# DJATOM/x265-aMod

Measured on AMD Instinct MI355X. Metric: encoded frames/sec at 1080p & 2160p --preset medium; bit-exact vs CPU ref, higher is better.
Workload: dtype u8

## Files before the change

### x265-amod_amd/csrc/encoder_api.hip

```cpp
#include "encoder_impl.h"

extern "C" void x265amd_param_default(x265amd_param* p)
{
    if (!p) return;
    memset(p, 0, sizeof(*p));
    p->fpsNum = 25; p->fpsDenom = 1;
    p->bframes = 0; p->keyframeMax = 250; p->maxNumReferences = 3; p->qp = 30; p->ipFactor = 1.4f; p->pbFactor = 1.3f;
    p->rateControlMode = X265AMD_RC_CQP; p->rfConstant = 28; p->aqStrength = 1.0; p->qCompress = 0.6; p->aqMode = 0; p->cuTree = 0; p->qgSize = 32; p->qpMin = 0; p->qpMax = 69; p->vuiVideoFormat = 5; p->vuiColorPrimaries = 2; p->vuiTransfer = 2; p->vuiMatrix = 2; p->bEmitCLL = 1;
    p->rdLevel = 3; p->limitReferences = 3; p->bEnableEarlySkip = 1; p->recursionSkipMode = 1; p->bIntraInBFrames = 1; p->psyRd = 2.0; p->edgeVarThreshold = 0.05f;
    p->searchMethod = X265AMD_ME_HEX; p->subpelRefine = 2; p->searchRange = 57; p->maxNumMergeCand = 3;
    p->bEnableSignHiding = 1; p->bEnableStrongIntraSmoothing = 1; p->bEnableTemporalMvp = 1; p->tuQTMaxInterDepth = 1; p->tuQTMaxIntraDepth = 1;
    p->bEnableLoopFilter = 1; p->bEnableSAO = 1; p->bEnableWavefront = 1; p->aspectRatioIdc = 0;
}

void x265amd_encoder::fillStreamParams(x265amd_stream_params& s) const
{
    memset(&s, 0, sizeof(s));
    static const struct { uint32_t maxLumaSamples, maxLumaSamplesPerSecond; int idc; } levels[] = {
        { 36864, 552960, 30 }, { 122880, 3686400, 60 }, { 245760, 7372800, 63 }, { 552960, 16588800, 90 }, { 983040, 33177600, 93 },
        { 2228224, 66846720, 120 }, { 2228224, 133693440, 123 }, { 8912896, 267386880, 150 }, { 8912896, 534773760, 153 },
        { 8912896, 1069547520, 156 }, { 35651584, 1069547520, 180 }, { 35651584, 2139095040u, 183 }, { 35651584, 4278190080u, 186 } };
    s.profile_idc = X265AMD_DEPTH <= 8 ? 1 : 2;
    s.profile_compatibility_flags = X265AMD_DEPTH <= 8 ? (1u << 1) | (1u << 2) : (1u << 2);
    s.progressive_source = 1; s.frame_only_constraint = 1;
    s.bit_depth_constraint = X265AMD_DEPTH; s.chroma_format_constraint = 1; s.lower_bit_rate_constraint = 1;
    s.intra_constraint = p.keyframeMax <= 1;
    if (s.intra_constraint) { s.profile_idc = 4; s.profile_compatibility_flags = 1u << 4; }
    const uint32_t lumaSamples = (uint32_t)(W * H);
    const uint32_t samplesPerSec = (uint32_t)(lumaSamples * ((double)p.fpsNum / p.fpsDenom));
    s.level_idc = 255;
    for (const auto& l : levels)
    {
        if (lumaSamples > l.maxLumaSamples || samplesPerSec > l.maxLumaSamplesPerSecond) continue;
        if (W > sqrt(l.maxLumaSamples * 8.0f) || H > sqrt(l.maxLumaSamples * 8.0f)) continue;
        uint32_t maxDpbSize = 6;
        if (lumaSamples <= (l.maxLumaSamples >> 2)) maxDpbSize = 16;
        else if (lumaSamples <= (l.maxLumaSamples >> 1)) maxDpbSize = 12;
        else if (lumaSamples <= ((3 * l.maxLumaSamples) >> 2)) maxDpbSize = 8;
        if ((uint32_t)maxDecPicBuffering > maxDpbSize) continue;
        s.level_idc = l.idc;
        break;
    }
    s.max_temporal_sub_layers = 1;
    s.max_dec_pic_buffering[0] = maxDecPicBuffering; s.num_reorder_pics[0] = numReorderPics; s.max_latency_increase[0] = p.bframes;
    s.chroma_format_idc = 1; s.pic_width = W; s.pic_height = H; s.bit_depth = X265AMD_DEPTH; s.log2_max_poc_lsb = 8;
    s.conformance_window = W != srcW || H != srcH; s.conf_win_offsets[1] = W - srcW; s.conf_win_offsets[3] = H - srcH;
    s.log2_min_cu_size = 3; s.log2_diff_max_min_cu_size = 3; s.tu_log2_min = 2; s.tu_log2_max = 5;
    s.tu_max_depth_inter = p.tuQTMaxInterDepth; s.tu_max_depth_intra = p.tuQTMaxIntraDepth;
    s.amp = p.bEnableAMP != 0; s.sao = p.bEnableSAO != 0; s.temporal_mvp = p.bEnableTemporalMvp != 0; s.strong_intra_smoothing = p.bEnableStrongIntraSmoothing != 0;
    s.aspect_ratio_idc = p.aspectRatioIdc; s.sar_width = p.vuiSarWidth; s.sar_height = p.vuiSarHeight;
    s.overscan_info_present = p.vuiOverscanInfoPresent != 0; s.overscan_appropriate = p.vuiOverscanAppropriate != 0;
    s.video_signal_type_present = p.vuiVideoSignalTypePresent != 0; s.video_format = p.vuiVideoFormat; s.video_full_range = p.vuiFullRange != 0;
    s.colour_description_present = p.vuiColorDescriptionPresent != 0; s.colour_primaries = p.vuiColorPrimaries; s.transfer_characteristics = p.vuiTransfer; s.matrix_coefficients = p.vuiMatrix;
    s.chroma_loc_info_present = p.vuiChromaLocPresent != 0; s.chroma_sample_loc_top = p.vuiChromaLocTop; s.chroma_sample_loc_bottom = p.vuiChromaLocBottom;
    s.default_display_window = p.vuiDisplayWindow != 0;
    s.def_disp_win_offsets[0] = p.vuiDispWinLeft; s.def_disp_win_offsets[1] = p.vuiDispWinRight; s.def_disp_win_offsets[2] = p.vuiDispWinTop; s.def_disp_win_offsets[3] = p.vuiDispWinBottom;
    s.emit_timing_info = 1; s.num_units_in_tick = p.fpsDenom; s.time_scale = p.fpsNum;
    s.weighted_pred = p.bEnableWeightedPred != 0; s.weighted_bipred = p.bEnableWeightedBiPred != 0;
    s.sign_hide = p.bEnableSignHiding != 0; s.num_ref_idx_default[0] = s.num_ref_idx_default[1] = 1; s.init_qp_minus26 = 0;
    s.use_dqp = useDqp; s.max_cu_dqp_depth = maxCuDqpDepth;
    s.wpp = p.bEnableWavefront != 0; s.loop_filter_across_slices = 1;
    s.deblocking_filter_control_present = !p.bEnableLoopFilter || p.deblockingFilterBetaOffset || p.deblockingFilterTCOffset; s.pic_disable_deblocking = !p.bEnableLoopFilter;
    s.beta_offset_div2 = p.deblockingFilterBetaOffset; s.tc_offset_div2 = p.deblockingFilterTCOffset;
}

extern "C" x265amd_encoder* x265amd_encoder_open(const x265amd_param* p)
{
    if (!p) { xa_fail(X265AMD_EINVAL, "encoder_open: null param"); return nullptr; }
    x265amd_param norm = *p;
    if (norm.keyframeMax < 0) { norm.keyframeMax = INT_MAX; norm.scenecutThreshold = 0; norm.bHistBasedSceneCut = 0; }
    if (norm.keyframeMax <= 1 && norm.keyframeMax >= 0)
    {
        norm.keyframeMax = 1; norm.keyframeMin = 1; norm.bFrameAdaptive = 0; norm.bframes = 0; norm.bOpenGOP = 0; norm.bRepeatHeaders = 1; norm.lookaheadDepth = 0;
        norm.scenecutThreshold = 0; norm.bHistBasedSceneCut = 0; norm.cuTree = 0; norm.bEnableWeightedPred = 0; norm.bEnableWeightedBiPred = 0; norm.maxNumReferences = 1;
    }
    if (norm.bEmitHDR10SEI || norm.hasMasteringDisplay || norm.maxCLL || norm.maxFALL) { norm.bEmitHDR10SEI = 1; norm.bRepeatHeaders = 1; }
    if (norm.limitTU && norm.tuQTMaxInterDepth < 2) norm.limitTU = 0;
    if (norm.rateControlMode != X265AMD_RC_CRF) { norm.aqMode = 0; norm.cuTree = 0; }
    if (norm.lookaheadDepth == 0) norm.cuTree = 0;
    if (!norm.aqMode && norm.cuTree) { norm.aqMode = 1; norm.aqStrength = 0.0; }
    if (norm.aqStrength == 0 && !norm.cuTree) norm.aqMode = 0;
    if ((((norm.sourceHeight + 7) & ~7) + 63) / 64 == 1 || (((norm.sourceWidth + 7) & ~7) + 63) / 64 < 3) norm.bEnableWavefront = 0;
    p = &norm;
    if (p->sourceWidth < 16 || p->sourceHeight < 16 || (p->sourceWidth & 1) || (p->sourceHeight & 1) || p->sourceWidth > 8192 || p->sourceHeight > 4320)
    { xa_fail(X265AMD_EINVAL, "encoder_open: picture size must be even (4:2:0) and within 16..8192 x 16..4320"); return nullptr; }
    if (p->sourceWidth <= 64 && p->sourceHeight <= 64)
    { xa_fail(X265AMD_EINVAL, "encoder_open: sourceWidth / sourceHeight: a picture of a single CTU is not built"); return nullptr; }
    {
        static thread_local char why[160];
        const char* bad = nullptr;
#define XA_REQUIRE(cond, text) do { if (!bad && !(cond)) bad = text; } while (0)
        XA_REQUIRE(p->fpsNum && p->fpsDenom, "fpsNum / fpsDenom must be non-zero");
        XA_REQUIRE(p->bframes >= 0 && p->bframes <= 16, "bframes outside 0..16");
        XA_REQUIRE(p->keyframeMax >= 1, "keyframeMax below 1");
        XA_REQUIRE(p->maxNumReferences >= 1 && p->maxNumReferences <= 8, "maxNumReferences outside 1..8");
        XA_REQUIRE(p->rateControlMode == 0 || p->rateControlMode == X265AMD_RC_CQP || p->rateControlMode == X265AMD_RC_CRF, "rc.rateControlMode: constant QP (1) and constant rate factor (2) are built, ABR (0 with a bitrate) is not");
        XA_REQUIRE(p->rateControlMode == X265AMD_RC_CRF || (p->qp >= 0 && p->qp <= 51), "qp outside 0..51");
        XA_REQUIRE(p->rateControlMode != X265AMD_RC_CRF || (p->rfConstant >= 0 && p->rfConstant <= 51), "rfConstant outside 0..51");
        XA_REQUIRE(p->aqMode >= 0 && p->aqMode <= 5, "aqMode outside 0..5");
        XA_REQUIRE(p->qpMin >= 0 && p->qpMin <= p->qpMax && p->qpMax <= 69, "qpMin / qpMax outside 0..69 (or crossed)");
        XA_REQUIRE(p->aspectRatioIdc >= 0 && (p->aspectRatioIdc <= 16 || p->aspectRatioIdc == 255), "aspectRatioIdc outside 0..16 / 255");
        XA_REQUIRE(p->deblockingFilterTCOffset >= -6 && p->deblockingFilterTCOffset <= 6 && p->deblockingFilterBetaOffset >= -6 && p->deblockingFilterBetaOffset <= 6, "deblocking offsets outside -6..6");
        XA_REQUIRE(p->limitTU == 0 || (p->limitTU >= 2 && p->limitTU <= 4), "limitTU: 0, 2, 3 and 4 are built (1, the breadth-first form, is not)");
        XA_REQUIRE(p->limitTU < 3 || p->shardCount <= 1, "limitTU 3 / 4 with pictures coded on several GPUs is not built (the transform depth records do not travel)");
        XA_REQUIRE(p->decodedPictureHashSEI >= 0 && p->decodedPictureHashSEI <= 3 && p->maxCLL >= 0 && p->maxCLL <= 65535 && p->maxFALL >= 0 && p->maxFALL <= 65535, "decodedPictureHashSEI outside 0..3 or a light level outside 16 bits");
        XA_REQUIRE(p->vuiVideoFormat >= 0 && p->vuiVideoFormat <= 5 && p->vuiColorPrimaries >= 0 && p->vuiColorPrimaries <= 255 && p->vuiTransfer >= 0 && p->vuiTransfer <= 255 &&
                   p->vuiMatrix >= 0 && p->vuiMatrix <= 255 && p->vuiChromaLocTop >= 0 && p->vuiChromaLocTop <= 5 && p->vuiChromaLocBottom >= 0 && p->vuiChromaLocBottom <= 5, "vui: a value outside its range");
        XA_REQUIRE(!p->aqMode || p->aqStrength >= 0, "aqStrength negative");
        XA_REQUIRE(!p->aqMode || p->qgSize == 32 || p->qgSize == 64, "qgSize: 64 and 32 are built");
        XA_REQUIRE(!p->cuTree || p->aqMode, "cuTree needs adaptive quantisation (Encoder::configure switches it on with cuTree; say aqMode)");
        XA_REQUIRE(!p->cuTree || p->rateControlMode == X265AMD_RC_CRF, "cuTree needs rate control (the reference switches it off under constant QP, encoder.cpp:3721-3728)");
        XA_REQUIRE(!p->cuTree || p->lookaheadDepth > 0, "cuTree needs the lookahead (lookaheadDepth > 0)");
        XA_REQUIRE(!(p->aqMode && p->rateControlMode != X265AMD_RC_CRF), "adaptive quantisation needs rate control (the reference switches it off under constant QP, encoder.cpp:3721-3728)");
        XA_REQUIRE(p->rdLevel >= 2 && p->rdLevel <= 6, "rdLevel outside 2..6 (rd 0-1 are not built)");
        XA_REQUIRE(p->maxNumMergeCand >= 1 && p->maxNumMergeCand <= 5, "maxNumMergeCand outside 1..5");
        XA_REQUIRE(p->tuQTMaxInterDepth >= 1 && p->tuQTMaxInterDepth <= 4, "tuQTMaxInterDepth outside 1..4");
        XA_REQUIRE(p->tuQTMaxIntraDepth >= 1 && p->tuQTMaxIntraDepth <= 4, "tuQTMaxIntraDepth outside 1..4");
        XA_REQUIRE(p->searchMethod == X265AMD_ME_DIA || p->searchMethod == X265AMD_ME_HEX || p->searchMethod == X265AMD_ME_STAR || p->searchMethod == X265AMD_ME_FULL, "searchMethod: only dia, hex, star and full are built (no umh / sea)");
        XA_REQUIRE(p->subpelRefine >= 0 && p->subpelRefine <= 7, "subpelRefine outside 0..7");
        XA_REQUIRE(p->rdoqLevel >= 0 && p->rdoqLevel <= 2, "rdoqLevel outside 0..2");
        XA_REQUIRE(p->psyRdoqFix8 >= 0, "psyRdoqFix8 negative");
        XA_REQUIRE(p->recursionSkipMode >= 0 && p->recursionSkipMode <= 2, "recursionSkipMode outside 0..2");
        XA_REQUIRE(p->recursionSkipMode != 2 || p->aqMode < 4, "recursionSkipMode 2 with aqMode 4 / 5 is not built (the bit plane would come from the filtered edge picture)");
        XA_REQUIRE(p->recursionSkipMode != 2 || (p->edgeVarThreshold >= 0.0f && p->edgeVarThreshold <= 1.0f), "edgeVarThreshold outside 0..1 (--rskip-edge-threshold 0..100)");
        XA_REQUIRE(p->recursionSkipMode != 2 || p->shardCount <= 1, "recursionSkipMode 2 with pictures coded on several GPUs (shardCount > 1) is not built");
        XA_REQUIRE(!p->bHistBasedSceneCut || X265AMD_DEPTH == 8, "bHistBasedSceneCut: histogram scene-cut detection is built for the 8-bit library only");
        XA_REQUIRE(!p->bHistBasedSceneCut || p->shardCount <= 1, "bHistBasedSceneCut with pictures coded on several GPUs (shardCount > 1) is not built");
        XA_REQUIRE(p->limitReferences >= 0 && p->limitReferences <= 3, "limitReferences outside 0..3");
        XA_REQUIRE(!p->bEnableAMP || p->bEnableRectInter, "bEnableAMP needs bEnableRectInter");
#undef XA_REQUIRE
        if (bad) { snprintf(why, sizeof(why), "encoder_open: %s", bad); xa_fail(X265AMD_EINVAL, why); return nullptr; }
    }
    xa_bind_device();
    std::unique_ptr<x265amd_encoder> e(new x265amd_encoder);
    e->p = *p;
    e->srcW = p->sourceWidth; e->srcH = p->sourceHeight;
    e->W = (p->sourceWidth + 7) & ~7; e->H = (p->sourceHeight + 7) & ~7; e->w4 = e->W / 4; e->h4 = e->H / 4;
    e->ctuW = (e->W + 63) / 64; e->ctuH = (e->H + 63) / 64; e->nctu = e->ctuW * e->ctuH;
    e->stride = e->W + 2 * e->marginX; e->cstride = e->W / 2 + e->marginX;
    const size_t ysz = (size_t)(e->H + 2 * e->marginY) * e->stride, csz = (size_t)(e->H / 2 + e->marginY) * e->cstride;
    e->org[0] = (size_t)e->marginY * e->stride + e->marginX;
    e->org[1] = ysz + (size_t)(e->marginY / 2) * e->cstride + e->marginX / 2;
    e->org[2] = ysz + csz + (size_t)(e->marginY / 2) * e->cstride + e->marginX / 2;
    e->picElems = ysz + 2 * csz;
    const double ipOffset = 6.0 * log2(p->ipFactor), pbOffset = 6.0 * log2(p->pbFactor);
    auto clipQp = [](int q) { return q < 0 ? 0 : q > 69 ? 69 : q; };
    e->qpConstant[1] = p->qp;
    e->qpConstant[2] = clipQp((int)(p->qp - ipOffset + 0.5));
    e->qpConstant[0] = clipQp((int)(p->qp + pbOffset + 0.5));
    if (e->qpConstant[0] > 51 || e->qpConstant[2] > 51) { xa_fail(X265AMD_EINVAL, "encoder_open: slice QP above 51"); return nullptr; }
    e->numReorderPics = (p->bBPyramid && p->bframes > 1) ? 2 : (p->bframes ? 1 : 0);
    e->maxDecPicBuffering = std::min(16, std::max(e->numReorderPics + 2, p->maxNumReferences) + 1);
    if (p->firstFrame < 0) { xa_fail(X265AMD_EINVAL, "encoder_open: firstFrame"); return nullptr; }
    e->frameCount = p->firstFrame; e->lastKeyframe = p->firstFrame - p->keyframeMax; e->lastIDR = p->firstFrame;
    if (p->scenecutThreshold < 0 || p->scenecutThreshold > 100 || p->lookaheadDepth < 0 || p->lookaheadDepth > 250 || p->keyframeMin < 0 || p->keyframeMin > p->keyframeMax)
    { xa_fail(X265AMD_EINVAL, "encoder_open: scenecutThreshold outside 0..100, lookaheadDepth outside 0..250 or keyframeMin outside 0..keyframeMax"); return nullptr; }
    if (p->shardCount < 0 || p->shardCount > 64 || (p->shardCount > 1 && (p->shardRank < 0 || p->shardRank >= p->shardCount || p->frameNumThreads <= 1)))
    { xa_fail(X265AMD_EINVAL, "encoder_open: shardRank / shardCount (frame-per-GPU needs 0 <= rank < count and frameNumThreads > 1: rows are published by pictures coded in parallel)"); return nullptr; }
    if (p->bFrameAdaptive < 0 || p->bFrameAdaptive > 2) { xa_fail(X265AMD_EINVAL, "encoder_open: bFrameAdaptive: 0 (fixed mini-GOPs), 1 (fast) or 2 (trellis)"); return nullptr; }
    e->lookahead = p->scenecutThreshold > 0 || p->bHistBasedSceneCut || (p->bFrameAdaptive && p->bframes) || p->cuTree || p->aqMode;
    x265amd_hist_scene_state_init(&e->histState);
    if ((p->bEnableWeightedPred || p->bEnableWeightedBiPred) && !e->lookahead) { xa_fail(X265AMD_EINVAL, "encoder_open: bEnableWeightedPred needs the lookahead (scenecutThreshold > 0 or bFrameAdaptive 2 with B frames)"); return nullptr; }
    {
        int kmin = p->keyframeMin;
        if (!kmin) { const double fps = (double)p->fpsNum / p->fpsDenom; kmin = std::min((int)fps, p->keyframeMax / 10); }
        e->keyframeMin = std::max(1, kmin);
        e->lowCuW = (e->W / 2 + 7) >> 3; e->lowCuH = (e->H / 2 + 7) >> 3;
        if (p->lookaheadSlices > 1 && e->H >= 720)
        {
            e->laRowsPerSlice = std::min(std::max(e->lowCuH / p->lookaheadSlices, 10), e->lowCuH);
            e->laNumSlices = e->lowCuH / e->laRowsPerSlice;
        }
        if (e->laNumSlices > 1 && p->bframes == 0 && p->lookaheadDepth > 0)
        { xa_fail(X265AMD_EINVAL, "encoder_open: bframes 0 with lookaheadSlices above 1 in a picture of 720 rows or more is not built (lookaheadSlices 0 is)"); return nullptr; }
        e->lowW = e->lowCuW * 8; e->lowH = e->lowCuH * 8;
        e->lowBlocks = (e->lowCuW > 2 && e->lowCuH > 2) ? (e->lowCuW - 2) * (e->lowCuH - 2) : e->lowCuW * e->lowCuH;
        e->lowStride = e->W / 2 + 2 * e->marginX;
        e->lowStride += (32 - (e->lowStride & 31)) & 31;
        e->lowPlaneElems = (size_t)(e->lowH + 2 * e->marginY) * e->lowStride;
        e->lowOrg = (size_t)e->marginY * e->lowStride + e->marginX;
        if (e->lookahead)
        {
            int least = 0, greatest = 0;
            if (hipDeviceGetStreamPriorityRange(&least, &greatest) != hipSuccess || least == greatest || hipStreamCreateWithPriority(&e->laStream, hipStreamNonBlocking, least) != hipSuccess)
                if (hipStreamCreateWithFlags(&e->laStream, hipStreamNonBlocking) != hipSuccess) { xa_fail(X265AMD_EHIP, "encoder_open: stream"); return nullptr; }
        }
    }
    {
        const char* ft = xa_env_str("X265AMD_FRAME_THREADS");
        e->frameThreads = ft ? atoi(ft) : 3;
        if (e->frameThreads < 1) e->frameThreads = 1;
    }
    if (p->frameNumThreads < 0 || p->frameNumThreads > 16) { xa_fail(X265AMD_EINVAL, "encoder_open: frameNumThreads"); return nullptr; }
    e->frameParallel = p->frameNumThreads > 1;
    const int queues = xa_queues_hint(0);
    if (e->frameParallel)
    {
        static const int hpelIters[8] = { 1, 1, 1, 2, 3, 1, 2, 3 };
        int range = p->searchRange;
        range += p->searchMethod < 2;
        range += 8 / 2;
        range += 2 + (hpelIters[p->subpelRefine] + 1) / 2;
        e->refLagRows = 1 + ((range + 63) / 64);
        if (!xa_env_present("X265AMD_FRAME_THREADS"))
        {
            const int rowsInFlight = p->bEnableWavefront ? std::max(1, std::min(e->ctuH, (e->ctuW + 1) / 2)) : 1;
            e->frameThreads = std::max(2, std::min(16, (queues > 0 ? queues : 16) / rowsInFlight));
        }
    }
    e->me = x265amd_me_open();
    if (!e->me) return nullptr;
    e->laPool.reset(new LaPool);
    e->laPool->one = (((size_t)e->lowCuW * e->lowCuH * 4) + 255) & ~(size_t)255;
    e->aqOn = p->aqMode != 0 && p->rateControlMode == X265AMD_RC_CRF;
    e->useDqp = e->aqOn;
    e->maxCuDqpDepth = e->aqOn ? (p->qgSize == 64 ? 0 : 1) : 0;
    memset(&e->treeParams, 0, sizeof(e->treeParams));
    e->treeParams.width8 = e->lowCuW; e->treeParams.height8 = e->lowCuH; e->treeParams.fps_num = p->fpsNum; e->treeParams.fps_denom = p->fpsDenom;
    e->treeParams.b_pyramid = p->bBPyramid != 0; e->treeParams.weighted_bipred = p->bEnableWeightedBiPred != 0; e->treeParams.lookahead_depth = p->lookaheadDepth;
    e->treeParams.strength = 5.0 * (1.0 - p->qCompress);
    if (p->rateControlMode == X265AMD_RC_CRF)
    {
        x265amd_rc_params rp;
        memset(&rp, 0, sizeof(rp));
        rp.width = e->W; rp.height = e->H; rp.fps_num = p->fpsNum; rp.fps_denom = p->fpsDenom; rp.bframes = p->bframes; rp.keyframe_max = p->keyframeMax; rp.cu_tree = p->cuTree != 0;
        rp.qp_min = p->qpMin; rp.qp_max = p->qpMax; rp.rf_constant = p->rfConstant; rp.q_compress = p->qCompress; rp.ip_factor = p->ipFactor; rp.pb_factor = p->pbFactor;
        e->rateCtl = x265amd_rc_open(&rp);
        if (!e->rateCtl) { xa_fail(X265AMD_EINVAL, "encoder_open: rate control parameters"); return nullptr; }
    }
    const size_t nstat = (size_t)e->nctu * 3 * 5 * 32;
    if (hipMalloc((void**)&e->dSaoCount, nstat * 4) != hipSuccess || hipMalloc((void**)&e->dSaoOrg, nstat * 4) != hipSuccess ||
        hipMalloc((void**)&e->dSaoParams, sizeof(x265amd_sao_ctu) * e->nctu) != hipSuccess ||
        hipMalloc((void**)&e->dDbUnits, sizeof(x265amd_deblock_unit) * e->w4 * e->h4) != hipSuccess ||
        xa_scratch_alloc((void**)&e->dSaoTmp, e->picElems * sizeof(pixel)) != hipSuccess)
    { xa_fail(X265AMD_EHIP, "encoder_open: device allocation"); return nullptr; }
    x265amd_stream_params sp;
    e->fillStreamParams(sp);
    e->headerBytes.resize(512);
    const size_t n = x265amd_write_stream_headers(&sp, e->headerBytes.data(), e->headerBytes.size());
    if (!n || n > e->headerBytes.size()) { xa_fail(X265AMD_EINVAL, "encoder_open: stream headers"); return nullptr; }
    e->headerBytes.resize(n);
    if (p->bEmitHDR10SEI || p->hasMasteringDisplay || p->maxCLL || p->maxFALL)
    {
        uint8_t sei[64], payload[24];
        if (p->bEmitCLL)
        {
            payload[0] = (uint8_t)(p->maxCLL >> 8); payload[1] = (uint8_t)p->maxCLL; payload[2] = (uint8_t)(p->maxFALL >> 8); payload[3] = (uint8_t)p->maxFALL;
            const size_t m = x265amd_write_sei(0, 144, payload, 4, sei, sizeof(sei));
            if (!m) { xa_fail(X265AMD_EINVAL, "encoder_open: content light level SEI"); return nullptr; }
            e->headerBytes.insert(e->headerBytes.end(), sei, sei + m);
        }
        if (p->hasMasteringDisplay)
        {
            for (int i = 0; i < 8; i++) { payload[2 * i] = (uint8_t)(p->masteringDisplay[i] >> 8); payload[2 * i + 1] = (uint8_t)p->masteringDisplay[i]; }
            for (int i = 0; i < 2; i++)
                for (int k = 0; k < 4; k++) payload[16 + 4 * i + k] = (uint8_t)(p->masteringDisplay[8 + i] >> (24 - 8 * k));
            const size_t m = x265amd_write_sei(0, 137, payload, 24, sei, sizeof(sei));
            if (!m) { xa_fail(X265AMD_EINVAL, "encoder_open: mastering display SEI"); return nullptr; }
            e->headerBytes.insert(e->headerBytes.end(), sei, sei + m);
        }
    }
    if (p->bEmitInfoSEI)
    {
        char text[1024];
        snprintf(text, sizeof(text), "x265amd (x265 build 209 interface) - %s - H.265/HEVC codec on AMD Instinct MI355X - options: %dx%d fps=%u/%u bitdepth=%d %s=%g aq-mode=%d aq-strength=%.2f "
                 "cutree=%d qcomp=%.2f qg-size=%d bframes=%d b-adapt=%d b-pyramid=%d open-gop=%d keyint=%d min-keyint=%d scenecut=%d rc-lookahead=%d lookahead-slices=%d ref=%d limit-refs=%d "
                 "rd=%d rdoq-level=%d psy-rd=%.2f me=%d subme=%d merange=%d max-merge=%d rect=%d amp=%d limit-modes=%d early-skip=%d rskip=%d weightp=%d weightb=%d sao=%d deblock=%d wpp=%d "
                 "tu-intra-depth=%d tu-inter-depth=%d signhide=%d strong-intra-smoothing=%d temporal-mvp=%d b-intra=%d fast-intra=%d",
                 x265amd_version(), p->sourceWidth, p->sourceHeight, p->fpsNum, p->fpsDenom, X265AMD_DEPTH, p->rateControlMode == X265AMD_RC_CRF ? "crf" : "qp",
                 p->rateControlMode == X265AMD_RC_CRF ? p->rfConstant : (double)p->qp, e->aqOn ? p->aqMode : 0, p->aqStrength, p->cuTree != 0, p->qCompress, p->qgSize, p->bframes, p->bFrameAdaptive,
                 p->bBPyramid != 0, p->bOpenGOP != 0, p->keyframeMax, e->keyframeMin, p->scenecutThreshold, p->lookaheadDepth, p->lookaheadSlices, p->maxNumReferences, p->limitReferences,
                 p->rdLevel, p->rdoqLevel, p->psyRd, p->searchMethod, p->subpelRefine, p->searchRange, p->maxNumMergeCand, p->bEnableRectInter != 0, p->bEnableAMP != 0, p->limitModes != 0,
                 p->bEnableEarlySkip != 0, p->recursionSkipMode, p->bEnableWeightedPred != 0, p->bEnableWeightedBiPred != 0, p->bEnableSAO != 0, p->bEnableLoopFilter != 0, p->bEnableWavefront != 0,
                 p->tuQTMaxIntraDepth, p->tuQTMaxInterDepth, p->bEnableSignHiding != 0, p->bEnableStrongIntraSmoothing != 0, p->bEnableTemporalMvp != 0, p->bIntraInBFrames != 0, p->bEnableFastIntra != 0);
        uint8_t sei[1400];
        const size_t m = x265amd_write_info_sei(text, sei, sizeof(sei));
        if (!m) { xa_fail(X265AMD_EINVAL, "encoder_open: info SEI"); return nullptr; }
        e->headerBytes.insert(e->headerBytes.end(), sei, sei + m);
    }
    return e.release();
}

static PicP picByCoding(x265amd_encoder* e, uint64_t k)
{
    std::lock_guard<std::mutex> lk(e->byCodingMu);
    auto it = e->byCoding.find(k);
    return it == e->byCoding.end() ? PicP() : it->second;
}
static void rowRanges(const x265amd_encoder& e, int row, uint64_t off[3], uint64_t bytes[3])
{
    for (int k = 0; k < 3; k++)
    {
        const int sh = k ? 1 : 0, my = e.marginY >> sh, mx = e.marginX >> sh, h = e.H >> sh, rowH = 64 >> sh;
        const intptr_t st = k ? e.cstride : e.stride;
        const int y0 = row == 0 ? -my : row * rowH, y1 = row == e.ctuH - 1 ? h + my : std::min(h, (row + 1) * rowH);
        const int64_t first = (int64_t)e.org[k] + (int64_t)y0 * st - mx;
        off[k] = (uint64_t)first * sizeof(pixel);
        bytes[k] = (uint64_t)((int64_t)(y1 - y0) * st) * sizeof(pixel);
    }
}
extern "C" int x265amd_encoder_ctu_rows(const x265amd_encoder* e) { return e ? e->ctuH : -1; }
extern "C" int x265amd_encoder_stats(const x265amd_encoder* e, uint64_t* out, int n)
{
    if (!e || !out || n < 4) return xa_fail(X265AMD_EINVAL, "encoder_stats: arguments"), -1;
    out[0] = e->statPictures[0]; out[1] = e->statPictures[1]; out[2] = e->statPictures[2]; out[3] = e->statReferences;
    if (n >= 13)
        for (int t = 0; t < 3; t++) { out[4 + t] = e->statEmitted[t]; out[7 + t] = e->statBits[t]; memcpy(&out[10 + t], &e->statQpSum[t], 8); }
    return 0;
}
extern "C" int x265amd_encoder_row_geometry(const x265amd_encoder* e, int row, x265amd_row_export* out)
{
    if (!e || !out || row < 0 || row >= e->ctuH) return xa_fail(X265AMD_EINVAL, "encoder_row_geometry: bad arguments"), -1;
    memset(out, 0, sizeof(*out));
    out->ctu_row = row;
    rowRanges(*e, row, out->plane_offset, out->plane_bytes);
    const size_t u0 = (size_t)row * 16 * e->w4, u1 = (size_t)std::min(e->h4, (row + 1) * 16) * e->w4;
    out->units_bytes = (u1 - u0) * sizeof(x265amd_cu_unit); out->map_offset_units = u0 * sizeof(x265amd_cu_unit);
    out->motion_bytes = (u1 - u0) * sizeof(x265amd_mv_unit); out->map_offset_motion = u0 * sizeof(x265amd_mv_unit);
    return 0;
}
extern "C" int x265amd_encoder_is_referenced(x265amd_encoder* e, uint64_t k)
{
    if (!e) return xa_fail(X265AMD_EINVAL, "encoder_is_referenced: null"), -1;
    PicP pic = picByCoding(e, k);
    if (!pic)
    {
        std::lock_guard<std::mutex> lk(e->byCodingMu);
        if (k < e->collectedCoding) return xa_fail(X265AMD_EINVAL, "encoder_is_referenced: that picture has been collected and released"), -1;
        return 2;
    }
    return pic->type != TYPE_B;
}
extern "C" int x265amd_encoder_owns(const x265amd_encoder* e, uint64_t k) { return e ? (e->p.shardCount <= 1 || (int)(k % (uint64_t)e->p.shardCount) == e->p.shardRank) : 0; }
extern "C" int x265amd_encoder_export_row(x265amd_encoder* e, uint64_t codingIndex, int row, x265amd_row_export* out, int timeoutMs)
{
    if (!e || !out || row < 0 || row >= e->ctuH) return xa_fail(X265AMD_EINVAL, "encoder_export_row: bad arguments"), -1;
    if (!e->frameParallel) return xa_fail(X265AMD_EINVAL, "encoder_export_row: rows are published by objects that code pictures in parallel (frameNumThreads > 1)"), -1;
    PicP pic = picByCoding(e, codingIndex);
    if (!pic)
    {
        std::lock_guard<std::mutex> lk(e->byCodingMu);
        if (codingIndex < e->collectedCoding) return xa_fail(X265AMD_EINVAL, "encoder_export_row: that picture has been collected and released: the pump is more than eight pictures late"), -1;
        return 1;
    }
    if (!pic->owned) return xa_fail(X265AMD_EINVAL, "encoder_export_row: this object does not code that picture"), -1;
    const auto t0 = std::chrono::steady_clock::now();
    while (pic->published(row) < e->W)
    {
        if (pic->failed.load()) return xa_fail(X265AMD_EHIP, "encoder_export_row: the picture failed"), -1;
        if (timeoutMs <= 0) return 2;
        if (std::chrono::duration<double, std::milli>(std::chrono::steady_clock::now() - t0).count() > timeoutMs) return xa_fail(X265AMD_EHIP, "encoder_export_row: time-out"), -1;
        std::this_thread::sleep_for(std::chrono::microseconds(200));
    }
    if (pic->failed.load()) return xa_fail(X265AMD_EHIP, "encoder_export_row: the picture failed"), -1;
    memset(out, 0, sizeof(*out));
    out->coding_index = codingIndex; out->ctu_row = row;
    rowRanges(*e, row, out->plane_offset, out->plane_bytes);
    for (int k = 0; k < 3; k++) out->src[k] = (const uint8_t*)pic->finalPlanes() + out->plane_offset[k];
    const size_t u0 = (size_t)row * 16 * e->w4, u1 = (size_t)std::min(e->h4, (row + 1) * 16) * e->w4;
    out->units = pic->units.data() + u0; out->units_bytes = (u1 - u0) * sizeof(x265amd_cu_unit); out->map_offset_units = u0 * sizeof(x265amd_cu_unit);
    out->motion = pic->motion.data() + u0; out->motion_bytes = (u1 - u0) * sizeof(x265amd_mv_unit); out->map_offset_motion = u0 * sizeof(x265amd_mv_unit);
    return 0;
}
extern "C" int x265amd_encoder_import_row(x265amd_encoder* e, const x265amd_row_export* in)
{
    if (!e || !in || in->ctu_row < 0 || in->ctu_row >= e->ctuH || !in->src[0] || !in->src[1] || !in->src[2] || !in->units || !in->motion) return xa_fail(X265AMD_EINVAL, "encoder_import_row: bad arguments"), -1;
    PicP pic = picByCoding(e, in->coding_index);
    if (!pic)
    {
        std::lock_guard<std::mutex> lk(e->byCodingMu);
        if (in->coding_index < e->collectedCoding) return xa_fail(X265AMD_EINVAL, "encoder_import_row: that picture has been collected and released"), -1;
        return 1;
    }
    if (pic->owned) return xa_fail(X265AMD_EINVAL, "encoder_import_row: this object codes that picture itself"), -1;
    uint64_t off[3], bytes[3];
    rowRanges(*e, in->ctu_row, off, bytes);
    for (int k = 0; k < 3; k++)
        if (off[k] != in->plane_offset[k] || bytes[k] != in->plane_bytes[k]) return xa_fail(X265AMD_EINVAL, "encoder_import_row: the row comes from a picture of another geometry"), -1;
    if (in->map_offset_units + in->units_bytes > pic->units.size() * sizeof(x265amd_cu_unit) || in->map_offset_motion + in->motion_bytes > pic->motion.size() * sizeof(x265amd_mv_unit))
        return xa_fail(X265AMD_EINVAL, "encoder_import_row: map range"), -1;
    xa_thread_device();
    uint8_t* dst = (uint8_t*)(pic->dFin ? pic->dFin : pic->dRec);
    {
        std::lock_guard<std::mutex> lk(e->importMu);
        if (!e->importStream && hipStreamCreateWithFlags(&e->importStream, hipStreamNonBlocking) != hipSuccess) return xa_fail(X265AMD_EHIP, "encoder_import_row: stream"), -1;
        for (int k = 0; k < 3; k++)
            if (hipMemcpyAsync(dst + off[k], in->src[k], bytes[k], hipMemcpyDefault, e->importStream) != hipSuccess) { pic->fail(); return xa_fail(X265AMD_EHIP, "encoder_import_row: copy"), -1; }
        if (hipStreamSynchronize(e->importStream) != hipSuccess) { pic->fail(); return xa_fail(X265AMD_EHIP, "encoder_import_row: copy"), -1; }
    }
    memcpy((uint8_t*)pic->units.data() + in->map_offset_units, in->units, in->units_bytes);
    memcpy((uint8_t*)pic->motion.data() + in->map_offset_motion, in->motion, in->motion_bytes);
    xa_devmap_push_rows(pic->motion.data(), pic->units.data(), e->w4, in->ctu_row * 16, std::min(e->h4, (in->ctu_row + 1) * 16));
    pic->publish(in->ctu_row, e->W);
    { std::lock_guard<std::mutex> lk(pic->mu); pic->importedRows++; }
    pic->cv.notify_all();
    return 0;
}

extern "C" void x265amd_encoder_close(x265amd_encoder* e) { delete e; }

static void splitNals(std::vector<uint8_t>& bytes, std::vector<x265amd_nal>& nals)
{
    nals.clear();
    std::vector<size_t> starts;
    for (size_t i = 0; i + 3 <= bytes.size(); i++)
        if (!bytes[i] && !bytes[i + 1] && bytes[i + 2] == 1) { starts.push_back(i > 0 && !bytes[i - 1] && (starts.empty() || starts.back() + 3 <= i - 1) ? i - 1 : i); i += 2; }
    for (size_t k = 0; k < starts.size(); k++)
    {
        const size_t start = starts[k], end = k + 1 < starts.size() ? starts[k + 1] : bytes.size();
        const size_t hdr = start + (bytes[start + 2] == 1 ? 3 : 4);
        x265amd_nal n;
        n.type = (bytes[hdr] >> 1) & 63; n.sizeBytes = (uint32_t)(end - start); n.payload = bytes.data() + start;
        nals.push_back(n);
    }
}

extern "C" int x265amd_encoder_headers(x265amd_encoder* e, x265amd_nal** ppNal, uint32_t* piNal)
{
    if (!e || !ppNal || !piNal) return xa_fail(X265AMD_EINVAL, "encoder_headers: null argument");
    e->outBytes = e->headerBytes;
    splitNals(e->outBytes, e->nals);
    *ppNal = e->nals.data(); *piNal = (uint32_t)e->nals.size();
    return (int)e->outBytes.size();
}

int x265amd_encoder::uploadPicture(const x265amd_picture* in, Pic& pic, bool onDevice)
{
    if (onDevice)
    {
        if (xa_scratch_alloc((void**)&pic.dSrc, picElems * sizeof(pixel)) != hipSuccess || xa_scratch_alloc((void**)&pic.dRec, picElems * sizeof(pixel)) != hipSuccess)
            return xa_fail(X265AMD_EHIP, "encoder_encode: device allocation");
        if (hipMemsetAsync(pic.dSrc, 0, picElems * sizeof(pixel), nullptr) != hipSuccess) return xa_fail(X265AMD_EHIP, "encoder_encode: memset");
        for (int k = 0; k < 3; k++)
        {
            const int w = k ? W / 2 : W, h = k ? H / 2 : H, mx = k ? marginX / 2 : marginX, my = k ? marginY / 2 : marginY;
            const intptr_t st = k ? cstride : stride;
            const int sw = k ? srcW / 2 : srcW, sh = k ? srcH / 2 : srcH;
            if (!in->planes[k] || in->stride[k] < (int)(sw * sizeof(pixel))) return xa_fail(X265AMD_EINVAL, "encoder_encode: input plane");
            if (hipMemcpy2DAsync(pic.dSrc + org[k], (size_t)st * sizeof(pixel), in->planes[k], (size_t)in->stride[k], (size_t)sw * sizeof(pixel), (size_t)sh, hipMemcpyDeviceToDevice, nullptr) != hipSuccess)
                return xa_fail(X265AMD_EHIP, "encoder_encode: the input picture is not device memory of this device");
            if ((sw != w || sh != h) && x265amd_extend_pic_border(nullptr, (x265amd_pixel*)(pic.dSrc + org[k]), st, sw, sh, w - sw, h - sh) != X265AMD_OK) return -1;
            if (x265amd_extend_pic_border(nullptr, (x265amd_pixel*)(pic.dSrc + org[k]), st, w, h, mx, my) != X265AMD_OK) return -1;
        }
        if (hipMemsetAsync(pic.dRec, 0, picElems * sizeof(pixel), nullptr) != hipSuccess) return xa_fail(X265AMD_EHIP, "encoder_encode: memset");
        if (frameParallel && p.bEnableSAO)
        {
            if (xa_scratch_alloc((void**)&pic.dFin, picElems * sizeof(pixel)) != hipSuccess) return xa_fail(X265AMD_EHIP, "encoder_encode: device allocation");
            if (hipMemsetAsync(pic.dFin, 0, picElems * sizeof(pixel), nullptr) != hipSuccess) return xa_fail(X265AMD_EHIP, "encoder_encode: memset");
        }
        if (hipStreamSynchronize(nullptr) != hipSuccess) return xa_fail(X265AMD_EHIP, "encoder_encode: the input picture's copy");
        return 0;
    }
    if (!uploadBuf)
    {
        if (hipHostMalloc((void**)&uploadBuf, picElems * sizeof(pixel), hipHostMallocDefault) != hipSuccess) { uploadBuf = nullptr; return xa_fail(X265AMD_EHIP, "encoder_encode: pinned input buffer"); }
        memset(uploadBuf, 0, picElems * sizeof(pixel));
    }
    for (int k = 0; k < 3; k++)
    {
        const int w = k ? W / 2 : W, h = k ? H / 2 : H, mx = k ? marginX / 2 : marginX, my = k ? marginY / 2 : marginY;
        const intptr_t st = k ? cstride : stride;
        const int sw = k ? srcW / 2 : srcW, sh = k ? srcH / 2 : srcH;
        if (!in->planes[k] || in->stride[k] < (int)(sw * sizeof(pixel))) return xa_fail(X265AMD_EINVAL, "encoder_encode: input plane");
        pixel* base = uploadBuf + org[k];
        for (int y = 0; y < h; y++)
        {
            const pixel* src = (const pixel*)((const uint8_t*)in->planes[k] + (size_t)(y < sh ? y : sh - 1) * in->stride[k]);
            pixel* row = base + (intptr_t)y * st;
            memcpy(row, src, sizeof(pixel) * sw);
            for (int x = sw; x < w; x++) row[x] = row[sw - 1];
            for (int x = 1; x <= mx; x++) { row[-x] = row[0]; row[w - 1 + x] = row[w - 1]; }
        }
        for (int y = 1; y <= my; y++)
        {
            memcpy(base + (intptr_t)(-y) * st - mx, base - mx, sizeof(pixel) * (w + 2 * mx));
            memcpy(base + (intptr_t)(h - 1 + y) * st - mx, base + (intptr_t)(h - 1) * st - mx, sizeof(pixel) * (w + 2 * mx));
        }
    }
    if (xa_scratch_alloc((void**)&pic.dSrc, picElems * sizeof(pixel)) != hipSuccess || xa_scratch_alloc((void**)&pic.dRec, picElems * sizeof(pixel)) != hipSuccess)
        return xa_fail(X265AMD_EHIP, "encoder_encode: device allocation");
    if (hipMemcpy(pic.dSrc, uploadBuf, picElems * sizeof(pixel), hipMemcpyHostToDevice) != hipSuccess) return xa_fail(X265AMD_EHIP, "encoder_encode: upload");
    if (hipMemset(pic.dRec, 0, picElems * sizeof(pixel)) != hipSuccess || hipStreamSynchronize(nullptr) != hipSuccess) return xa_fail(X265AMD_EHIP, "encoder_encode: memset");
    if (frameParallel && p.bEnableSAO)
    {
        if (xa_scratch_alloc((void**)&pic.dFin, picElems * sizeof(pixel)) != hipSuccess) return xa_fail(X265AMD_EHIP, "encoder_encode: device allocation");
        if (hipMemset(pic.dFin, 0, picElems * sizeof(pixel)) != hipSuccess || hipStreamSynchronize(nullptr) != hipSuccess) return xa_fail(X265AMD_EHIP, "encoder_encode: memset");
    }
    return 0;
}

static int encoder_encode_impl(x265amd_encoder* e, x265amd_nal** ppNal, uint32_t* piNal, const x265amd_picture* picIn, x265amd_picture* picOut, bool inputOnDevice);
extern "C" int x265amd_encoder_encode(x265amd_encoder* e, x265amd_nal** ppNal, uint32_t* piNal, const x265amd_picture* picIn, x265amd_picture* picOut)
{
    return encoder_encode_impl(e, ppNal, piNal, picIn, picOut, false);
}
extern "C" int x265amd_encoder_encode_device(x265amd_encoder* e, x265amd_nal** ppNal, uint32_t* piNal, const x265amd_picture* picIn, x265amd_picture* picOut)
{
    return encoder_encode_impl(e, ppNal, piNal, picIn, picOut, true);
}
static int encoder_encode_impl(x265amd_encoder* e, x265amd_nal** ppNal, uint32_t* piNal, const x265amd_picture* picIn, x265amd_picture* picOut, bool inputOnDevice)
{
    if (!e) return xa_fail(X265AMD_EINVAL, "encoder_encode: null encoder");
    if (ppNal) *ppNal = nullptr;
    if (piNal) *piNal = 0;
    if (picIn)
    {
        PicP pic(new Pic);
        pic->pool = e->laPool;
        pic->poc = e->frameCount++;
        const auto tu0 = std::chrono::steady_clock::now();
        int rc = e->uploadPicture(picIn, *pic, inputOnDevice);
        if (rc) return -1;
        const auto tl0 = std::chrono::steady_clock::now();
        e->uploadMs += std::chrono::duration<double, std::milli>(tl0 - tu0).count();
        if (e->lookahead && (rc = e->lowresInit(*pic)) != X265AMD_OK) return -1;
        e->laInitMs += std::chrono::duration<double, std::milli>(std::chrono::steady_clock::now() - tl0).count();
        e->input.push_back(pic);
    }
    const bool flushing = picIn == nullptr;
    auto decide = [e, flushing]() -> int {
        const auto tl1 = std::chrono::steady_clock::now();
        int rc = X265AMD_OK;
        if (e->lookahead) rc = e->decideLookahead(flushing, flushing ? 1 : 1 << 30);
        else e->decideMiniGop(flushing);
        const double ms = std::chrono::duration<double, std::milli>(std::chrono::steady_clock::now() - tl1).count();
        e->laDecideMs += ms;
        static const bool timingD = xa_env_present("X265AMD_TIMING");
        if (timingD && ms > 0.5) fprintf(stderr, "x265amd: decision: %.1f ms, %d pictures typed, %d still in the lookahead%s\n", ms, (int)e->ready.size(), (int)e->input.size(), flushing ? " (flushing)" : "");
        return rc;
    };
    auto admit = [e]() -> int {
        while (!e->ready.empty())
        {
            PicP pic = e->ready.front();
            e->ready.pop_front();
            if (e->prepare(pic)) return -1;
            pic->codingOrder = e->codingCount++;
            pic->owned = e->p.shardCount <= 1 || (int)(pic->codingOrder % (uint64_t)e->p.shardCount) == e->p.shardRank;
            e->inflight.push_back(pic);
            { std::lock_guard<std::mutex> lk(e->byCodingMu); e->byCoding[pic->codingOrder] = pic; }
        }
        return 0;
    };
    if (decide() != X265AMD_OK || admit()) return -1;
    const bool timing = xa_env_present("X265AMD_TIMING");
    auto start = [e, timing](const PicP& pic) {
        std::shared_future<int> prev = e->lastTask;
        pic->started = true;
        if (timing) fprintf(stderr, "x265amd: poc %d handed to a frame task at %.1f ms (%d running)\n", pic->poc, Pic::pubClockMs(), e->running);
        pic->done = std::async(std::launch::async, [e, pic, prev, timing]() {
            xa_thread_device();
            const auto t0 = std::chrono::steady_clock::now();
            if (!pic->owned)
            {
                if (pic->type == TYPE_B) { if (!e->keepSources()) { xa_scratch_free(pic->dSrc); pic->dSrc = nullptr; } return (int)X265AMD_OK; }
                std::unique_lock<std::mutex> lk(pic->mu);
                static const int importWaitS = xa_env_int("X265AMD_IMPORT_WAIT_S", 300);
                const bool ok = pic->cv.wait_for(lk, std::chrono::seconds(importWaitS), [&] { return pic->importedRows >= e->ctuH || pic->failed.load(); });
                if (!ok || pic->failed.load()) { lk.unlock(); pic->fail(); return xa_fail(X265AMD_EHIP, "encoder: a picture coded elsewhere did not arrive"); }
                lk.unlock();
                if (!e->keepSources()) { xa_scratch_free(pic->dSrc); pic->dSrc = nullptr; }
                return (int)X265AMD_OK;
            }
            const int rc = e->frameParallel ? e->runFrameParallel(pic) : e->runFrame(pic, prev);
            { struct timespec ts; clock_gettime(CLOCK_THREAD_CPUTIME_ID, &ts); e->cpuPictureNs += (uint64_t)ts.tv_sec * 1000000000ull + (uint64_t)ts.tv_nsec; }
            if (timing)
                fprintf(stderr, "x265amd: poc %d type %d qp %d: %.2f ms\n", pic->poc, pic->type, pic->sliceQp,
                        std::chrono::duration<double, std::milli>(std::chrono::steady_clock::now() - t0).count());
            return rc;
        }).share();
        e->lastTask = pic->done;
        e->running++;
    };
    const int earlyPMax = 6;
    const int earlyBMax = e->ctuH > 24 ? 12 : 0;
    auto launch = [&]() {
    const bool headLong = !e->inflight.empty() && (e->inflight.front()->type == TYPE_IDR || e->inflight.front()->type == TYPE_I) && e->inflight.front()->started &&
                          e->inflight.front()->done.wait_for(std::chrono::seconds(0)) != std::future_status::ready;
    for (auto& q : e->inflight)
    {
        if (q->started) continue;
        if (e->running <= e->frameThreads || q == e->inflight.front()) { start(q); if (e->frameThreads <= 1) q->done.wait(); continue; }
        if (!e->frameParallel) break;
        if (q->type == TYPE_IDR || q->type == TYPE_I) start(q);
        else if (headLong && q->type == TYPE_P && e->running <= e->frameThreads + earlyPMax) start(q);
        else if (earlyBMax > 0 && headLong && e->running <= e->frameThreads + earlyBMax) start(q);
    }
    };
    launch();
    while (flushing && !e->input.empty())
    {
        if (!e->inflight.empty() && e->inflight.front()->started && e->inflight.front()->done.wait_for(std::chrono::seconds(0)) == std::future_status::ready) break;
        const size_t before = e->input.size();
        if (decide() != X265AMD_OK || admit()) return -1;
        launch();
        if (e->input.size() >= before) break;
    }
    if (e->inflight.empty()) return 0;
    PicP front = e->inflight.front();
    if (!front->started) { xa_fail(X265AMD_EINVAL, "encoder_encode: the first picture in coding order has no task"); return -1; }
    int waiting = 0;
    for (auto& q : e->inflight) waiting += !q->started;
    const bool mustWait = !picIn || (e->running > e->frameThreads && waiting > 2 * e->p.lookaheadDepth + 8);
    if (!mustWait && front->done.wait_for(std::chrono::seconds(0)) != std::future_status::ready) return 0;
    const int rc = front->done.get();
    e->inflight.pop_front();
    e->running--;
    {
        std::lock_guard<std::mutex> lk(e->byCodingMu);
        e->collectedCoding = front->codingOrder + 1;
        while (!e->byCoding.empty() && e->byCoding.begin()->first + 8 < e->collectedCoding) e->byCoding.erase(e->byCoding.begin());
    }
    if (rc) { xa_fail(rc, "encoder_encode: a frame task failed"); return -1; }
    if (const char* dumpPath = xa_env_str("X265AMD_RC_DUMP"))
    {
        if (FILE* f = fopen(dumpPath, "ab"))
        {
            const Pic& q = *front;
            const int blocks16 = ((e->W + 15) / 16) * ((e->H + 15) / 16), lowresBlocks = e->lowCuW * e->lowCuH;
            int32_t hdr[44];
            memset(hdr, 0, sizeof(hdr));
            hdr[0] = 0x52434450; hdr[1] = q.poc; hdr[2] = q.type; hdr[3] = q.type != TYPE_B; hdr[4] = q.sliceQp; hdr[5] = q.bScenecut;
            for (int l = 0; l < 2; l++) { hdr[6 + l] = (int32_t)q.lists[l].size(); for (size_t r = 0; r < q.lists[l].size() && r < 16; r++) hdr[8 + 16 * l + r] = q.lists[l][r]->poc; }
            hdr[40] = e->w4; hdr[41] = e->h4; hdr[42] = blocks16; hdr[43] = lowresBlocks;
            fwrite(hdr, sizeof(hdr), 1, f);
            const int64_t satd = 0; fwrite(&satd, 8, 1, f);
            const double qq[2] = { q.avgQpRc, 0 }; fwrite(qq, 8, 2, f);
            std::vector<double> zd((size_t)blocks16, 0.0); std::vector<int32_t> zi((size_t)std::max(blocks16, lowresBlocks), 0); std::vector<uint16_t> zs((size_t)lowresBlocks, 0);
            fwrite(q.qpAqOffset.size() == (size_t)blocks16 ? q.qpAqOffset.data() : zd.data(), 8, blocks16, f);
            fwrite(q.qpCuTreeOffset.size() == (size_t)blocks16 ? q.qpCuTreeOffset.data() : zd.data(), 8, blocks16, f);
            fwrite(q.invQscale.size() == (size_t)blocks16 ? q.invQscale.data() : zi.data(), 4, blocks16, f);
            fwrite(q.intraCostHost.size() == (size_t)lowresBlocks ? q.intraCostHost.data() : zi.data(), 4, lowresBlocks, f);
            fwrite(q.propagateCost.size() == (size_t)lowresBlocks ? q.propagateCost.data() : zs.data(), 2, lowresBlocks, f);
            const size_t n = (size_t)e->w4 * e->h4;
            std::vector<uint8_t> b(n);
            for (size_t i = 0; i < n; i++) b[i] = (uint8_t)q.units[i].qp; fwrite(b.data(), 1, n, f);
            for (size_t i = 0; i < n; i++) b[i] = q.units[i].depth; fwrite(b.data(), 1, n, f);
            for (size_t i = 0; i < n; i++) b[i] = q.units[i].pred_mode; fwrite(b.data(), 1, n, f);
            for (size_t i = 0; i < n; i++) b[i] = q.units[i].cbf[0]; fwrite(b.data(), 1, n, f);
            fclose(f);
        }
    }
    e->outBytes.swap(front->nalBytes);
    const bool withAud = e->p.bEnableAccessUnitDelimiters && (front->poc || e->p.bRepeatHeaders) && !e->outBytes.empty();
    const bool withHeaders = e->p.bRepeatHeaders && front->bKeyframe && !e->outBytes.empty();
    if (withAud || withHeaders)
    {
        std::vector<uint8_t> au;
        if (withAud)
        {
            uint8_t aud[16];
            const size_t m = x265amd_write_aud(isBType(front->type) ? 0 : front->type == TYPE_P ? 1 : 2, aud, sizeof(aud));
            au.insert(au.end(), aud, aud + m);
        }
        if (withHeaders) au.insert(au.end(), e->headerBytes.begin(), e->headerBytes.end());
        const std::vector<uint8_t>& b = e->outBytes;
        for (size_t i = 0; i < b.size(); i++)
        {
            if (i + 4 <= b.size() && !b[i] && !b[i + 1] && !b[i + 2] && b[i + 3] == 1) continue;
            au.push_back(b[i]);
        }
        e->outBytes.swap(au);
    }
    bool haveStaging = false;
    if (e->p.decodedPictureHashSEI && !e->outBytes.empty())
    {
        e->staging.resize(e->picElems);
        if (hipMemcpy(e->staging.data(), front->finalPlanes(), e->picElems * sizeof(pixel), hipMemcpyDeviceToHost) != hipSuccess) { xa_fail(X265AMD_EHIP, "encoder: recon download"); return -1; }
        haveStaging = true;
        const void* planes[3] = { e->staging.data() + e->org[0], e->staging.data() + e->org[1], e->staging.data() + e->org[2] };
        const intptr_t strides[3] = { (intptr_t)(e->stride * sizeof(pixel)), (intptr_t)(e->cstride * sizeof(pixel)), (intptr_t)(e->cstride * sizeof(pixel)) };
        uint8_t payload[64], sei[96];
        const size_t n = x265amd_picture_hash(e->p.decodedPictureHashSEI, planes, strides, e->W, e->H, X265AMD_DEPTH, 64, payload, sizeof(payload));
        const size_t m = n ? x265amd_write_sei(1, 132, payload, n, sei, sizeof(sei)) : 0;
        if (!m) { xa_fail(X265AMD_EINVAL, "encoder: picture hash SEI"); return -1; }
        e->outBytes.insert(e->outBytes.end(), sei, sei + m);
    }
    splitNals(e->outBytes, e->nals);
    if (!e->outBytes.empty())
    {
        const int t = front->type == TYPE_B || front->type == TYPE_BREF ? 2 : (front->type == TYPE_P ? 1 : 0);
        const size_t n = (size_t)e->w4 * e->h4;
        double q = 0;
        if (e->useDqp && front->units.size() >= n) { int64_t sum = 0; for (size_t i = 0; i < n; i++) sum += front->units[i].qp; q = (double)sum / (double)n; }
        else q = front->sliceQp;
        e->statEmitted[t]++; e->statBits[t] += (uint64_t)e->outBytes.size() * 8; e->statQpSum[t] += q;
    }
    if (picOut)
    {
        e->staging.resize(e->picElems);
        if (!haveStaging && hipMemcpy(e->staging.data(), front->finalPlanes(), e->picElems * sizeof(pixel), hipMemcpyDeviceToHost) != hipSuccess) { xa_fail(X265AMD_EHIP, "encoder: recon download"); return -1; }
        for (int k = 0; k < 3; k++)
        {
            if (!picOut->planes[k]) continue;
            const int w = k ? e->srcW / 2 : e->srcW, hh = k ? e->srcH / 2 : e->srcH;
            const intptr_t st = k ? e->cstride : e->stride;
            for (int y = 0; y < hh; y++)
                memcpy((uint8_t*)picOut->planes[k] + (size_t)y * picOut->stride[k], e->staging.data() + e->org[k] + (intptr_t)y * st, sizeof(pixel) * w);
        }
        picOut->poc = front->poc; picOut->sliceType = front->type; picOut->qp = front->sliceQp;
    }
    front->lists[0].clear(); front->lists[1].clear(); front->neg.clear(); front->pos.clear();
    if (ppNal) *ppNal = e->nals.data();
    if (piNal) *piNal = (uint32_t)e->nals.size();
    return 1;
}
```

### x265-amod_amd/csrc/encoder_impl.h

```cpp
#ifndef X265AMD_ENCODER_IMPL_H
#define X265AMD_ENCODER_IMPL_H
#include <hip/hip_runtime.h>
#include "x265amd.h"
#include "x265amd_encoder.h"
#include "x265amd_host.h"
#include "x265amd_ratecontrol.h"
#include <immintrin.h>
#include "xa_fiber.h"
#include <limits.h>
#include <math.h>
#include <stdio.h>
#include <stdlib.h>
#include <chrono>
#include <string.h>
#include <algorithm>
#include <atomic>
#include <condition_variable>
#include <deque>
#include <map>
#include <mutex>
#include <thread>
#include <future>
#include <memory>
#include <vector>

namespace xaenc {

typedef x265amd_pixel pixel;
enum { TYPE_AUTO = 0, TYPE_IDR = 1, TYPE_I = 2, TYPE_P = 3, TYPE_BREF = 4, TYPE_B = 5 };
static inline bool isBType(int t) { return t == TYPE_B || t == TYPE_BREF; }
enum { RD_TILE_ELEMS = 4096 + 2 * 1024 };

struct LaPool
{
    std::mutex mu;
    size_t one = 0;
    std::vector<void*> freeBufs, chunks;
    ~LaPool() { for (void* c : chunks) (void)hipFree(c); }
    void* get()
    {
        std::lock_guard<std::mutex> lk(mu);
        if (freeBufs.empty())
        {
            void* chunk = nullptr;
            if (!one || hipMalloc(&chunk, one * 64) != hipSuccess) return nullptr;
            chunks.push_back(chunk);
            for (int i = 63; i >= 0; i--) freeBufs.push_back((char*)chunk + one * i);
        }
        void* p = freeBufs.back();
        freeBufs.pop_back();
        return p;
    }
    void put(void* p) { if (!p) return; std::lock_guard<std::mutex> lk(mu); freeBufs.push_back(p); }
    std::vector<const void*> deadFields;
    void dead(const void* key) { if (!key) return; std::lock_guard<std::mutex> lk(mu); deadFields.push_back(key); }
};

struct Pic;
typedef std::shared_ptr<Pic> PicP;
struct Pic
{
    int poc = 0, type = 0, sliceQp = 0;
    uint64_t codingOrder = 0;
    bool started = false;
    bool owned = true;
    int importedRows = 0;
    bool hasReferences = false;
    pixel* dSrc = nullptr; pixel* dRec = nullptr;
    std::vector<x265amd_cu_unit> units;
    std::vector<x265amd_mv_unit> motion;
    int32_t refPoc[2][16];
    int nalType = 0, lastIDR = 0;
    bool rpsUsed = true;
    std::vector<PicP> neg, pos, lists[2];
    std::shared_future<int> done;
    std::vector<uint8_t> nalBytes;
    pixel* dFin = nullptr;
    std::mutex mu;
    std::condition_variable cv;
    int analysedRows = 0;
    std::vector<volatile uint64_t*> finalX;
    std::vector<int> analysedCols;
    std::atomic<bool> failed{ false };
    const pixel* finalPlanes() const { return dFin ? dFin : dRec; }
    pixel* dLowres = nullptr; int32_t* dIntraCost = nullptr;
    int64_t costEst[18]; int intraMbs[18];
    std::vector<int16_t> lowMvs[18];
    std::vector<int16_t> lowMvs1[18];
    std::vector<int32_t> lowMvc[18], lowMvc1[18];
    int64_t cost2[18][18];
    std::vector<int16_t> specMvs[18], specMvs1[18];
    std::vector<int32_t> specMvc[18], specMvc1[18];
    int64_t specCost2[18][18]; int specIntraMbs[18];
    uint64_t wpSum[3] = { 0, 0, 0 }, wpSsd[3] = { 0, 0, 0 };
    int lumaDenom = 7, chromaDenom = 7;
    x265amd_weight wp[2][16][3];
    bool weighted = false;
    bool bScenecut = false, bKeyframe = false;
    std::vector<int8_t> tuRecs;
    std::unique_ptr<x265amd_hist_scene_pic> hist;
    bool bHistScenecutAnalyzed = false;
    uint32_t* edgeCounts = nullptr;
    std::vector<int32_t> intraCostHost;
    std::vector<double> qpAqOffset, qpCuTreeOffset;
    std::vector<int32_t> invQscale;
    std::vector<uint16_t> propagateCost;
    std::map<int, void*> dLc, dSpecLc;
    std::map<int, std::vector<uint16_t> > lcHost;
    std::shared_ptr<LaPool> pool;
    void dropLc(std::map<int, void*>& m, int key) { auto it = m.find(key); if (it != m.end()) { if (pool) pool->put(it->second); m.erase(it); } }
    double avgQpRc = 0;
    bool bLastMiniGopBFrame = false;
    std::vector<int8_t> cuQp;
    const x265amd_mv_unit* regMotion = nullptr;
    void registerMotion()
    {
        if (regMotion == motion.data()) return;
        if (regMotion) xa_devmap_unregister(regMotion);
        regMotion = motion.data();
        if (!xa_devmap_register(regMotion, motion.size())) regMotion = nullptr;
    }
    Pic() { memset(refPoc, 0, sizeof(refPoc)); memset(wp, 0, sizeof(wp)); for (int i = 0; i < 18; i++) { costEst[i] = -1; intraMbs[i] = 0; specIntraMbs[i] = 0; for (int j = 0; j < 18; j++) cost2[i][j] = specCost2[i][j] = -1; } }
    ~Pic() { if (pool) { for (auto& e : dLc) pool->put(e.second); for (auto& e : dSpecLc) pool->put(e.second);
                         for (int i = 0; i < 18; i++) for (const std::vector<int16_t>* v : { &lowMvs[i], &lowMvs1[i], &specMvs[i], &specMvs1[i] }) if (!v->empty()) pool->dead(v->data()); } if (regMotion) xa_devmap_unregister(regMotion); xa_scratch_free(dSrc); xa_scratch_free(dRec); xa_scratch_free(dFin); xa_scratch_free(dLowres); xa_scratch_free(dIntraCost); if (edgeCounts) xa_mapped_free(edgeCounts); for (volatile uint64_t* c : finalX) xa_counter_free(c); }
    void publish(int row, int x)
    {
        std::atomic_thread_fence(std::memory_order_release); *finalX[row] = (uint64_t)x;
        static const bool pubLog = xa_env_present("X265AMD_PUB_LOG");
        if (pubLog) fprintf(stderr, "x265amd pub: poc %d row %d x %d at %.2f\n", poc, row, x, pubClockMs());
    }
    static double pubClockMs() { return fmod(std::chrono::duration<double, std::milli>(std::chrono::steady_clock::now().time_since_epoch()).count(), 1e6); }
    int published(int row) const { const int v = (int)*finalX[row]; std::atomic_thread_fence(std::memory_order_acquire); return v; }
    void fail()
    {
        failed.store(true, std::memory_order_release);
        for (volatile uint64_t* c : finalX) *c = 1u << 30;
        { std::lock_guard<std::mutex> lk(mu); }
        cv.notify_all();
    }
};

}
using namespace xaenc;

struct x265amd_encoder
{
    x265amd_param p;
    x265amd_me_ctx* me = nullptr;
    int W = 0, H = 0, w4 = 0, h4 = 0, ctuW = 0, ctuH = 0, nctu = 0;
    int srcW = 0, srcH = 0;
    int marginX = 96, marginY = 80;
    intptr_t stride = 0, cstride = 0;
    size_t org[3] = { 0, 0, 0 }, picElems = 0;
    int qpConstant[3] = { 0, 0, 0 };
    int maxDecPicBuffering = 0, numReorderPics = 0;
    int frameCount = 0, lastKeyframe = 0, lastIDR = 0;
    bool haveKeyframe = false, refreshPending = false;
    int pocCRA = 0;
    bool first = true;
    std::deque<PicP> input;
    std::deque<PicP> ready;
    std::deque<PicP> inflight;
    uint64_t codingCount = 0;
    int running = 0;
    std::mutex importMu;
    hipStream_t importStream = nullptr;
    std::mutex byCodingMu;
    std::map<uint64_t, PicP> byCoding;
    uint64_t collectedCoding = 0;
    uint64_t statPictures[3] = { 0, 0, 0 }, statReferences = 0;
    uint64_t statEmitted[3] = { 0, 0, 0 }, statBits[3] = { 0, 0, 0 }; double statQpSum[3] = { 0, 0, 0 };
    std::shared_future<int> lastTask;
    int frameThreads = 1;
    double uploadMs = 0;
    std::atomic<uint64_t> cpuPictureNs{ 0 }, cpuFilterNs{ 0 };
    bool frameParallel = false;
    int refLagRows = 0;
    std::vector<PicP> picList;
    double depthSaoRate[8] = { 0, 0, 0, 0, 0, 0, 0, 0 };
    std::vector<uint8_t> headerBytes, outBytes;
    std::vector<x265amd_nal> nals;
    std::vector<pixel> staging;
    pixel* uploadBuf = nullptr;
    int32_t* dSaoCount = nullptr; int32_t* dSaoOrg = nullptr; x265amd_sao_ctu* dSaoParams = nullptr; x265amd_deblock_unit* dDbUnits = nullptr;
    pixel* dSaoTmp = nullptr;

    ~x265amd_encoder()
    {
        for (auto& q : inflight) if (q->done.valid()) q->done.wait();
        laFieldsFree();
        if (uploadBuf) (void)hipHostFree(uploadBuf);
        if (xa_env_present("X265AMD_TIMING") && lookahead)
        {
            fprintf(stderr, "x265amd: input: %.1f ms in uploads; cpu of the picture threads %.1f ms, of the filter threads %.1f ms\n", uploadMs, cpuPictureNs.load() / 1e6, cpuFilterNs.load() / 1e6);
            fprintf(stderr, "x265amd: lookahead: %.1f ms in lowres planes + intra costs, %.1f ms in the slice-type decision (%llu estimates, %llu motion searches; %llu batches %.1f ms, %llu single estimates %.1f ms)\n", laInitMs, laDecideMs,
                    (unsigned long long)laJobs, (unsigned long long)laSearches, (unsigned long long)laBatches, laBatchMs, (unsigned long long)laSingles, laSingleMs);
            fprintf(stderr, "x265amd: lookahead estimates by phase: set-up %.1f ms, launch call %.1f, read-back issued %.1f, waited for %.1f, host sums %.1f; %llu weight guesses measured\n", laPhaseMs[0], laPhaseMs[1], laPhaseMs[2], laPhaseMs[3], laPhaseMs[4], (unsigned long long)laWeightJobs);
        }
        if (me) x265amd_me_close(me);
        if (rateCtl) x265amd_rc_close(rateCtl);
        if (dSaoCount) (void)hipFree(dSaoCount);
        if (dSaoOrg) (void)hipFree(dSaoOrg);
        if (dSaoParams) (void)hipFree(dSaoParams);
        if (dDbUnits) (void)hipFree(dDbUnits);
        xa_scratch_free(dSaoTmp);
        xa_scratch_free(histRecord);
        if (histRecordHost) xa_mapped_free(histRecordHost);
        if (laStream) (void)hipStreamDestroy(laStream);
        if (importStream) (void)hipStreamDestroy(importStream);
    }
    uint64_t planeAddr(const pixel* base, int k) const { return (uint64_t)(uintptr_t)(base + org[k]); }

    void fillStreamParams(x265amd_stream_params& s) const;
    int uploadPicture(const x265amd_picture* in, Pic& pic, bool onDevice = false);
    void decideMiniGop(bool flush);
    int prepare(const PicP& pic);
    int runFrame(const PicP& pic, std::shared_future<int> prev);
    int runFrameParallel(const PicP& pic);
    int edgeCounts(Pic& pic, hipStream_t st, x265amd_rskip_edge& edge);
    bool lookahead = false;
    void* wpEnergy = nullptr; void* wpSums = nullptr; void* wpSumsHost = nullptr; void* wpMvs = nullptr;
    int laRowsPerSlice = 0, laNumSlices = 1;
    int keyframeMin = 1, lowW = 0, lowH = 0, lowCuW = 0, lowCuH = 0, lowBlocks = 0;
    intptr_t lowStride = 0; size_t lowPlaneElems = 0, lowOrg = 0;
    PicP lastNonB;
    bool isSceneTransition = false;
    hipStream_t laStream = nullptr;
    int lowresInit(Pic& pic);
    void pushMiniGop(int b);
    struct LaWeight { int minscale = 0, mindenom = 0, curScale = 0, curOffset = 0; };
    bool lookaheadWeightGuess(Pic& fenc, Pic& ref, LaWeight& g);
    void lookaheadWeightDecide(const LaWeight& g, const uint32_t costs[2], bool& weighted, int& scale, int& denom, int& offset);
    int sliceWeights(Pic& pic);
    bool keepSources() const { return p.bEnableWeightedPred || p.bEnableWeightedBiPred; }
    int weightRows(struct WPlane& wpl, int r0, int r1);
    int frameCostP(Pic& b, Pic& ref, int dist);
    int frameCostAt(Pic& fenc, Pic& ref0, Pic* ref1, int d0, int d1, int64_t& score);
    struct CostJob { Pic* fenc = nullptr; Pic* ref0 = nullptr; Pic* ref1 = nullptr; int d0 = 0, d1 = 0; bool spec = false; bool whole = false; bool search0 = false, search1 = false; void* dMvs = nullptr; void* dMvc = nullptr; void* dMvs1 = nullptr;
                     void* dMvc1 = nullptr; void* dLc = nullptr; void* dBc = nullptr; void* dW = nullptr; };
    int frameCostMany(std::vector<CostJob>& jobs);
    struct DevField { void* mv; void* mc; uint64_t used; };
    std::map<const void*, DevField> laFields;
    uint64_t laFieldClock = 0;
    static const size_t LA_FIELDS_MAX = 2048;
    std::shared_ptr<LaPool> laPool;
    void* laBuf() { return laPool->get(); }
    void laBufPut(void* p) { laPool->put(p); }
    void laFieldPut(const void* key, void* mv, void* mc);
    void laFieldsTrim();
    void laFieldsFree();
    double laPhaseMs[5] = { 0, 0, 0, 0, 0 };
    double laInitMs = 0, laDecideMs = 0, laBatchMs = 0, laSingleMs = 0; uint64_t laJobs = 0, laSearches = 0, laBatches = 0, laSingles = 0, laWeightJobs = 0;
    int frameCost(std::vector<Pic*>& frames, int p0, int p1, int b, int64_t& score);
    int64_t planCost(std::vector<Pic*>& frames, const std::vector<uint8_t>& runs, int64_t limit, int& rc);
    void extendPlans(std::vector<Pic*>& frames, int length, std::vector<std::vector<uint8_t> >& plans, int& rc);
    bool scenecutInternal(std::vector<Pic*>& frames, int p0, int p1, bool real, int& rc);
    bool scenecut(std::vector<Pic*>& frames, int p0, int p1, bool real, int numFrames, int& rc);
    void* histRecord = nullptr; void* histRecordHost = nullptr;
    x265amd_hist_scene_state histState;
    bool histBasedScenecut(std::vector<Pic*>& frames, int p0, int p1, int numFrames);
    int slicetypeAnalyse(std::vector<Pic*>& frames, bool bKeyframe = false);
    int decideLookahead(bool flush, int maxGops = 1 << 30);
    x265amd_rc* rateCtl = nullptr;
    bool useDqp = false; int maxCuDqpDepth = 0;
    bool aqOn = false;
    void* aqEnergy = nullptr; void* aqEnergyHost = nullptr; void* aqSums = nullptr;
    x265amd_cutree_params treeParams;
    int adaptiveQuant(Pic& pic);
    int runCuTree(std::vector<Pic*>& frames, int numframes, bool bIntra);
    static int cuTreeEstimate(void* ctx, int p0, int p1, int b, const uint16_t** lc, const int16_t** mvs0, const int16_t** mvs1);
    int64_t estimatedPictureCost(Pic& pic);
    void cuQpTable(Pic& pic);
    int filterRows(Pic& pic, const x265amd_slice_info& si, const x265amd_mvpred_info& info, std::vector<x265amd_sao_ctu>& sparams, int32_t* saoFlags);
    int filterRowsCols(Pic& pic, const x265amd_slice_info& si, const x265amd_mvpred_info& info, std::vector<x265amd_sao_ctu>& sparams, int32_t* saoFlags);
};

#endif
```

### x265-amod_amd/csrc/encoder_lookahead.hip

```cpp
#include "encoder_impl.h"

int x265amd_encoder::lowresInit(Pic& pic)
{
    if (xa_scratch_alloc((void**)&pic.dLowres, lowPlaneElems * 4 * sizeof(pixel)) != hipSuccess || xa_scratch_alloc((void**)&pic.dIntraCost, (size_t)lowCuW * lowCuH * 4 + (size_t)lowCuW * lowCuH) != hipSuccess)
        return xa_fail(X265AMD_EHIP, "encoder_encode: device allocation");
    if (hipMemsetAsync(pic.dLowres, 0, lowPlaneElems * 4 * sizeof(pixel), laStream) != hipSuccess) return xa_fail(X265AMD_EHIP, "encoder_encode: memset");
    pixel* planes[4];
    for (int k = 0; k < 4; k++) planes[k] = pic.dLowres + (size_t)k * lowPlaneElems + lowOrg;
    int rc = x265amd_lowres_init(laStream, pic.dSrc + org[0], stride, lowW, lowH, planes, lowStride, marginX, marginY);
    if (rc != X265AMD_OK) return rc;
    const int lambda = X265AMD_DEPTH > 8 ? 16 : 1;
    uint8_t* dMode = (uint8_t*)(pic.dIntraCost + (size_t)lowCuW * lowCuH);
    rc = x265amd_lowres_intra_costs(laStream, planes[0], lowStride, lowCuW, lowCuH, lambda, pic.dIntraCost, dMode);
    if (rc != X265AMD_OK) return rc;
    static const char* const dbgWp = xa_env_str("X265AMD_WP_DEBUG");
    const bool sums = (p.bEnableWeightedPred || p.bEnableWeightedBiPred) && !(dbgWp && strchr(dbgWp, 's'));
    if (sums && !aqOn)
    {
        const int bw = (W + 15) / 16, bh = (H + 15) / 16;
        if (!wpEnergy && (xa_scratch_alloc(&wpEnergy, (size_t)bw * bh * 4) != hipSuccess || xa_scratch_alloc(&wpSums, 6 * 8) != hipSuccess || xa_mapped_alloc(&wpSumsHost, 6 * 8, true) != hipSuccess ||
                          xa_mapped_alloc(&wpMvs, (size_t)lowCuW * lowCuH * 4, false) != hipSuccess))
            return xa_fail(X265AMD_EHIP, "encoder_encode: device allocation");
        const uint64_t srcP[3] = { planeAddr(pic.dSrc, 0), planeAddr(pic.dSrc, 1), planeAddr(pic.dSrc, 2) };
        rc = x265amd_aq_energy(laStream, srcP, stride, cstride, W, H, 16, (uint32_t*)wpEnergy, (uint64_t*)wpSums);
        if (rc == X265AMD_OK && hipMemcpyAsync(wpSumsHost, wpSums, 6 * 8, hipMemcpyDeviceToHost, laStream) != hipSuccess) rc = xa_fail(X265AMD_EHIP, "encoder_encode: picture sums");
        if (rc != X265AMD_OK) return rc;
    }
    if (aqOn && (rc = adaptiveQuant(pic)) != X265AMD_OK) return rc;
    if (p.bHistBasedSceneCut)
    {
        const size_t bytes = X265AMD_HIST_SCENE_RECORD_BYTES(H);
        if (!histRecord && (xa_scratch_alloc(&histRecord, bytes) != hipSuccess || xa_mapped_alloc(&histRecordHost, bytes, true) != hipSuccess))
            return xa_fail(X265AMD_EHIP, "encoder_encode: device allocation");
        const uint64_t srcP[3] = { planeAddr(pic.dSrc, 0), planeAddr(pic.dSrc, 1), planeAddr(pic.dSrc, 2) };
        rc = x265amd_hist_scene_stats(laStream, srcP, stride, cstride, (uint64_t)(uintptr_t)planes[0], lowStride, W, H, (x265amd_hist_scene_record*)histRecord, 0);
        if (rc != X265AMD_OK) return rc;
        if (hipMemcpyAsync(histRecordHost, histRecord, bytes, hipMemcpyDeviceToHost, laStream) != hipSuccess) return xa_fail(X265AMD_EHIP, "encoder_encode: picture statistics");
    }
    std::vector<int32_t> ic((size_t)lowCuW * lowCuH);
    if (hipMemcpyAsync(ic.data(), pic.dIntraCost, ic.size() * 4, hipMemcpyDeviceToHost, laStream) != hipSuccess || hipStreamSynchronize(laStream) != hipSuccess)
        return xa_fail(X265AMD_EHIP, "encoder_encode: lowres intra costs");
    if (p.bHistBasedSceneCut)
    {
        pic.hist.reset(new x265amd_hist_scene_pic);
        if (x265amd_hist_scene_finish((const x265amd_hist_scene_record*)histRecordHost, W, H, pic.hist.get()) != X265AMD_OK) return xa_fail(X265AMD_EINVAL, "encoder_encode: picture statistics");
        pic.bHistScenecutAnalyzed = false;
    }
    if (aqOn)
    {
        const int bw = (W + 15) / 16, bh = (H + 15) / 16, nb = bw * bh;
        pic.qpAqOffset.assign((size_t)nb, 0.0); pic.qpCuTreeOffset.assign((size_t)nb, 0.0); pic.invQscale.assign((size_t)nb, 256);
        if (p.aqStrength != 0 && p.aqMode >= 4)
        {
            const uint32_t* density = (const uint32_t*)((const char*)aqEnergyHost + (size_t)nb * 4 + 6 * 8);
            rc = x265amd_aq_offsets_edge((const uint32_t*)aqEnergyHost, density, density + nb, nb, lowCuW * lowCuH, p.aqMode, p.aqStrength, 1.0, 16, pic.qpAqOffset.data(), pic.qpCuTreeOffset.data(), pic.invQscale.data());
        }
        else if (p.aqStrength != 0)
            rc = x265amd_aq_offsets((const uint32_t*)aqEnergyHost, nb, lowCuW * lowCuH, p.aqMode, p.aqStrength, 1.0, 16, pic.qpAqOffset.data(), pic.qpCuTreeOffset.data(), pic.invQscale.data());
        if (rc != X265AMD_OK) return xa_fail(rc, "encoder_encode: adaptive quantisation");
        pic.intraCostHost = ic;
        if (p.cuTree) pic.propagateCost.assign((size_t)lowCuW * lowCuH, 0);
    }
    int64_t est = 0;
    const bool all = lowCuW <= 2 || lowCuH <= 2;
    for (int y = 0; y < lowCuH; y++)
        for (int x = 0; x < lowCuW; x++)
            if (all || (x > 0 && x < lowCuW - 1 && y > 0 && y < lowCuH - 1)) est += ic[(size_t)y * lowCuW + x];
    pic.costEst[0] = est;
    if (sums)
    {
        uint64_t wp[6];
        memcpy(wp, aqOn ? (const void*)((const char*)aqEnergyHost + (size_t)((W + 15) / 16) * ((H + 15) / 16) * 4) : wpSumsHost, sizeof(wp));
        const int maxCol = ((W + 8) >> 4) << 4, maxRow = ((H + 8) >> 4) << 4;
        const int width[3] = { maxCol, maxCol >> 1, maxCol >> 1 }, height[3] = { maxRow, maxRow >> 1, maxRow >> 1 };
        for (int i = 0; i < 3; i++)
        {
            const uint64_t sum = wp[i], ssd = wp[3 + i];
            pic.wpSum[i] = sum;
            pic.wpSsd[i] = ssd - (sum * sum + (uint64_t)((width[i] * height[i]) / 2)) / (uint64_t)(width[i] * height[i]);
        }
    }
    return X265AMD_OK;
}

int x265amd_encoder::adaptiveQuant(Pic& pic)
{
    const int bw = (W + 15) / 16, bh = (H + 15) / 16;
    const size_t nb = (size_t)bw * bh;
    const bool edge = p.aqMode >= 4 && p.aqStrength != 0;
    const size_t perBlock = edge ? 12 : 4;
    if (!aqEnergy && (xa_scratch_alloc(&aqEnergy, nb * perBlock) != hipSuccess || xa_scratch_alloc(&aqSums, 6 * 8) != hipSuccess || xa_mapped_alloc(&aqEnergyHost, nb * perBlock + 6 * 8, true) != hipSuccess))
        return xa_fail(X265AMD_EHIP, "encoder_encode: device allocation");
    if ((p.bEnableWeightedPred || p.bEnableWeightedBiPred) && !wpMvs && xa_mapped_alloc(&wpMvs, (size_t)lowCuW * lowCuH * 4, false) != hipSuccess)
        return xa_fail(X265AMD_EHIP, "encoder_encode: device allocation");
    const uint64_t srcP[3] = { planeAddr(pic.dSrc, 0), planeAddr(pic.dSrc, 1), planeAddr(pic.dSrc, 2) };
    int rc = x265amd_aq_energy(laStream, srcP, stride, cstride, W, H, 16, (uint32_t*)aqEnergy, (uint64_t*)aqSums);
    if (rc != X265AMD_OK) return rc;
    if (edge)
    {
        uint32_t* density = (uint32_t*)aqEnergy + nb;
        rc = xa_aq_edge(laStream, srcP[0], stride, W, H, 16, density, density + nb, (uint64_t*)aqSums, (uint64_t*)aqSums + 3, 0, 0);
        if (rc != X265AMD_OK) return rc;
        if (hipMemcpyAsync((char*)aqEnergyHost + nb * 4 + 6 * 8, density, nb * 8, hipMemcpyDeviceToHost, laStream) != hipSuccess)
            return xa_fail(X265AMD_EHIP, "encoder_encode: edge densities");
    }
    if (hipMemcpyAsync(aqEnergyHost, aqEnergy, nb * 4, hipMemcpyDeviceToHost, laStream) != hipSuccess ||
        hipMemcpyAsync((char*)aqEnergyHost + nb * 4, aqSums, 6 * 8, hipMemcpyDeviceToHost, laStream) != hipSuccess)
        return xa_fail(X265AMD_EHIP, "encoder_encode: block energies");
    return X265AMD_OK;
}

namespace {
inline int bitSizeOf(unsigned v) { int n = 1; while (v > 1) { v >>= 1; n += 2; } return n; }
inline int bsSizeUe(unsigned val) { return bitSizeOf(val + 1); }
inline int bsSizeSe(int val) { int tmp = 1 - val * 2; if (tmp < 0) tmp = val * 2; return tmp < 256 ? bitSizeOf((unsigned)tmp) : bitSizeOf((unsigned)(tmp >> 8)) + 16; }
inline x265amd_weight_cand weightCand(int scale, int denom, int offset)
{
    const int correction = 14 - X265AMD_DEPTH;
    x265amd_weight_cand c;
    c.present = 1; c.w0 = scale; c.round = (denom ? 1 << (denom - 1) : 0) << correction; c.shift = denom + correction; c.offset = offset << (X265AMD_DEPTH - 8);
    return c;
}
}

bool x265amd_encoder::lookaheadWeightGuess(Pic& fenc, Pic& ref, LaWeight& g)
{
    static const float epsilon = 1.f / 128.f;
    float guessScale, fencMean, refMean;
    if (fenc.wpSsd[0] && ref.wpSsd[0]) guessScale = sqrtf((float)fenc.wpSsd[0] / ref.wpSsd[0]);
    else guessScale = 1.0f;
    fencMean = (float)fenc.wpSum[0] / (lowH * lowW) / (1 << (X265AMD_DEPTH - 8));
    refMean = (float)ref.wpSum[0] / (lowH * lowW) / (1 << (X265AMD_DEPTH - 8));
    if (fabsf(refMean - fencMean) < 0.5f && fabsf(1.f - guessScale) < epsilon) return false;
    {
        int w = (int)(guessScale * 128 + 0.5f), d = 7;
        while (d > 0 && w > 127) { d--; w >>= 1; }
        w = std::min(w, 127);
        g.mindenom = d; g.minscale = w;
    }
    g.curScale = g.minscale;
    g.curOffset = (int)(fencMean - refMean * g.curScale / (1 << g.mindenom) + 0.5f);
    if (g.curOffset < -128 || g.curOffset > 127)
    {
        g.curOffset = std::max(-128, std::min(127, g.curOffset));
        g.curScale = (int)((1 << g.mindenom) * (fencMean - g.curOffset) / refMean + 0.5f);
        g.curScale = std::max(0, std::min(127, g.curScale));
    }
    return true;
}
void x265amd_encoder::lookaheadWeightDecide(const LaWeight& g, const uint32_t costs[2], bool& weighted, int& scale, int& denom, int& offset)
{
    weighted = false;
    int minoff = 0, minscale = g.minscale, mindenom = g.mindenom;
    unsigned int minscore = costs[0], origscore = costs[0];
    int found = 0;
    if (!minscore) return;
    const unsigned int sc = costs[1];
    if (sc < minscore) { minscore = sc; minscale = g.curScale; minoff = g.curOffset; found = 1; }
    if (mindenom > 0 && !(minscale & 1))
    {
        const int idx = minscale ? __builtin_ctz((unsigned)minscale) : 32;
        const int shift = std::min(idx, mindenom);
        mindenom -= shift; minscale >>= shift;
    }
    if (!found || (minscale == 1 << mindenom && minoff == 0) || (float)minscore / origscore > 0.998f) return;
    weighted = true; scale = minscale; denom = mindenom; offset = minoff;
}
int x265amd_encoder::sliceWeights(Pic& pic)
{
    pic.weighted = false;
    memset(pic.wp, 0, sizeof(pic.wp));
    const int numDirs = isBType(pic.type) ? 2 : 1;
    const float epsilon = 1.f / 128.f;
    const int w16 = ((W + 15) >> 4) << 4, h16 = ((H + 15) >> 4) << 4;
    int numpixels[3];
    numpixels[0] = w16 * h16; numpixels[1] = numpixels[2] = numpixels[0] >> 2;
    auto setW = [](x265amd_weight& w, bool present, int scale, int denom, int off) { w.present = present; w.w = (int16_t)scale; w.denom = (uint8_t)denom; w.o = (int16_t)off; };
    int chromaDenom = 7, lumaDenom = 7;
    const int lambda = X265AMD_DEPTH > 8 ? 16 : 1;
    for (int list = 0; list < numDirs; list++)
    {
        x265amd_weight* weights = pic.wp[list][0];
        Pic& ref = *pic.lists[list][0];
        const int diffPoc = abs(pic.poc - ref.poc);
        float guessScale[3], fencMean[3], refMean[3];
        for (int plane = 0; plane < 3; plane++)
        {
            setW(weights[plane], false, 1, 0, 0);
            const uint64_t fencVar = pic.wpSsd[plane] + !ref.wpSsd[plane], refVar = ref.wpSsd[plane] + !ref.wpSsd[plane];
            guessScale[plane] = sqrt((float)fencVar / refVar);
            fencMean[plane] = (float)pic.wpSum[plane] / (numpixels[plane]) / (1 << (X265AMD_DEPTH - 8));
            refMean[plane] = (float)ref.wpSum[plane] / (numpixels[plane]) / (1 << (X265AMD_DEPTH - 8));
        }
        while (!list && chromaDenom > 0)
        {
            const float thresh = 127.f / (1 << chromaDenom);
            if (guessScale[1] < thresh && guessScale[2] < thresh) break;
            chromaDenom--;
        }
        setW(weights[1], false, 1 << chromaDenom, chromaDenom, 0);
        setW(weights[2], false, 1 << chromaDenom, chromaDenom, 0);
        void* dMvs = nullptr;
        for (int plane = 0; plane < 3; plane++)
        {
            const int denom = plane ? chromaDenom : lumaDenom;
            if (plane && !weights[0].present) break;
            if (fabsf(refMean[plane] - fencMean[plane]) < 0.5f && fabsf(1.f - guessScale[plane]) < epsilon) { setW(weights[plane], false, 1 << denom, denom, 0); continue; }
            if (plane)
            {
                const int scale = std::max(0, std::min(255, (int)(guessScale[plane] * (1 << denom) + 0.5f)));
                if (scale > 127) continue;
                weights[plane].w = (int16_t)scale;
            }
            else
            {
                int w = (int)(guessScale[plane] * (1 << denom) + 0.5f), d = denom;
                while (!list && d > 0 && w > 127) { d--; w >>= 1; }
                w = std::min(w, 127);
                weights[plane].o = 0; weights[plane].denom = (uint8_t)d; weights[plane].w = (int16_t)w;
            }
            int mindenom = weights[plane].denom, minscale = weights[plane].w, minoff = 0;
            if (!plane && diffPoc <= p.bframes + 1)
            {
                const std::vector<int16_t>& f = list ? pic.lowMvs1[diffPoc < 18 ? diffPoc : 0] : pic.lowMvs[diffPoc < 18 ? diffPoc : 0];
                if (diffPoc < 18 && !f.empty())
                {
                    if (!wpMvs || f.size() * 2 > (size_t)lowCuW * lowCuH * 4) return xa_fail(X265AMD_EHIP, "encoder_encode: lowres vectors");
                    dMvs = wpMvs;
                    memcpy(dMvs, f.data(), f.size() * 2);
                }
            }
            struct Cand { int scale, off, startOffset, iter; };
            std::vector<Cand> order;
            std::vector<x265amd_weight_cand> cands(1);
            memset(&cands[0], 0, sizeof(cands[0]));
            const int startScale = std::max(0, std::min(127, minscale - 4)), endScale = std::max(0, std::min(127, minscale + 4));
            for (int scale = startScale; scale <= endScale; scale++)
            {
                const int deltaWeight = scale - (1 << mindenom);
                if (deltaWeight > 127 || deltaWeight <= -128) continue;
                int curScale = scale;
                int curOffset = (int)(fencMean[plane] - refMean[plane] * curScale / (1 << mindenom) + 0.5f);
                if (curOffset < -128 || curOffset > 127)
                {
                    curOffset = std::max(-128, std::min(127, curOffset));
                    curScale = (int)((1 << mindenom) * (fencMean[plane] - curOffset) / refMean[plane] + 0.5f);
                    curScale = std::max(0, std::min(127, curScale));
                }
                const int startOffset = std::max(-128, std::min(127, curOffset - 2)), endOffset = std::max(-128, std::min(127, curOffset + 2));
                for (int off = startOffset; off <= endOffset; off++) { order.push_back({ curScale, off, startOffset, scale }); cands.push_back(weightCand(curScale, mindenom, off)); }
            }
            std::vector<uint32_t> costs(cands.size(), 0);
            int rc;
            if (!plane)
            {
                const pixel* refPlanes[4];
                for (int t = 0; t < 4; t++) refPlanes[t] = ref.dLowres + (size_t)t * lowPlaneElems + lowOrg;
                rc = x265amd_lowres_weight_costs(laStream, pic.dLowres + lowOrg, refPlanes, (const int16_t*)dMvs, pic.dIntraCost, lowStride, lowW, lowH, cands.data(), (int)cands.size(), costs.data());
            }
            else
            {
                if (!pic.dSrc || !ref.dSrc) return xa_fail(X265AMD_EHIP, "encoder_encode: weight analysis without the reference's source picture");
                const int cw = ((W >> 4) << 4) >> 1, chh = ((H >> 4) << 4) >> 1;
                rc = x265amd_chroma_weight_costs(laStream, pic.dSrc + org[plane], ref.dSrc + org[plane], (const int16_t*)dMvs, cstride, cw, chh, lowCuW, lowCuH, cands.data(), (int)cands.size(), costs.data());
            }
            if (rc != X265AMD_OK) return rc;
            const uint32_t origscore = costs[0];
            if (!origscore) { setW(weights[plane], false, 1 << denom, denom, 0); continue; }
            uint32_t minscore = origscore;
            bool bFound = false;
            for (size_t k = 0; k < order.size(); k++)
            {
                const Cand& c = order[k];
                const int lam = plane ? lambda * 4 : lambda;
                const int hdr = lam * (10 + bsSizeUe((unsigned)mindenom) * (plane ? 1 : 2) + 2 * (bsSizeSe(c.scale) + bsSizeSe(c.off)));
                const uint32_t sc = costs[k + 1] + (uint32_t)hdr;
                if (sc < minscore) { minscore = sc; minscale = c.scale; minoff = c.off; bFound = true; }
                if (minoff == c.startOffset && c.off != c.startOffset)
                    while (k + 1 < order.size() && order[k + 1].iter == c.iter) k++;
            }
            if (!(plane || list) && mindenom > 0 && !(minscale & 1))
            {
                const int idx = minscale ? __builtin_ctz((unsigned)minscale) : 32;
                const int shift = std::min(idx, mindenom);
                mindenom -= shift; minscale >>= shift;
            }
            if (!bFound || (minscale == (1 << mindenom) && minoff == 0) || (float)minscore / origscore > 0.998f) setW(weights[plane], false, 1 << denom, denom, 0);
            else setW(weights[plane], true, minscale, mindenom, minoff);
        }
        if (weights[0].present && weights[1].present != weights[2].present)
        {
            if (weights[1].present) weights[2] = weights[1]; else weights[1] = weights[2];
        }
        lumaDenom = weights[0].denom; chromaDenom = weights[1].denom;
        for (size_t r = 1; r < pic.lists[list].size(); r++)
        {
            setW(pic.wp[list][r][0], false, 1 << lumaDenom, lumaDenom, 0);
            setW(pic.wp[list][r][1], false, 1 << chromaDenom, chromaDenom, 0);
            setW(pic.wp[list][r][2], false, 1 << chromaDenom, chromaDenom, 0);
        }
        for (int plane = 0; plane < 3; plane++) pic.weighted |= weights[plane].present != 0;
    }
    pic.lumaDenom = pic.wp[0][0][0].denom; pic.chromaDenom = pic.wp[0][0][1].denom;
    const bool wpLog = xa_env_present("X265AMD_WP_LOG");
    if (wpLog && pic.weighted)
    {
        char buf[512]; int n = snprintf(buf, sizeof(buf), "poc: %d weights:", pic.poc);
        for (int list = 0; list < numDirs; list++)
        {
            const x265amd_weight* w = pic.wp[list][0];
            if (!(w[0].present || w[1].present || w[2].present)) continue;
            n += snprintf(buf + n, sizeof(buf) - n, " [L%d:R0 ", list);
            if (w[0].present) n += snprintf(buf + n, sizeof(buf) - n, "Y{%d/%d%+d}", w[0].w, 1 << w[0].denom, w[0].o);
            if (w[1].present) n += snprintf(buf + n, sizeof(buf) - n, "U{%d/%d%+d}", w[1].w, 1 << w[1].denom, w[1].o);
            if (w[2].present) n += snprintf(buf + n, sizeof(buf) - n, "V{%d/%d%+d}", w[2].w, 1 << w[2].denom, w[2].o);
            n += snprintf(buf + n, sizeof(buf) - n, "]");
        }
        fprintf(stderr, "x265amd: %s\n", buf);
    }
    return X265AMD_OK;
}

int x265amd_encoder::frameCostP(Pic& b, Pic& ref, int dist)
{
    int64_t score;
    return frameCostAt(b, ref, nullptr, dist, 0, score);
}

int x265amd_encoder::frameCostAt(Pic& fenc, Pic& ref0, Pic* ref1, int d0, int d1, int64_t& score)
{
    if (d0 < 1 || d0 > 17 || d1 < 0 || d1 > 17 || (d1 > 0) != (ref1 != nullptr)) return xa_fail(X265AMD_EINVAL, "encoder: lookahead distance");
    if (fenc.cost2[d0][d1] >= 0) { score = fenc.cost2[d0][d1]; return X265AMD_OK; }
    if (fenc.lowMvs[d0].empty() && !fenc.specMvs[d0].empty()) { fenc.lowMvs[d0].swap(fenc.specMvs[d0]); fenc.lowMvc[d0].swap(fenc.specMvc[d0]); }
    if (d1 > 0 && fenc.lowMvs1[d1].empty() && !fenc.specMvs1[d1].empty()) { fenc.lowMvs1[d1].swap(fenc.specMvs1[d1]); fenc.lowMvc1[d1].swap(fenc.specMvc1[d1]); }
    if (fenc.specCost2[d0][d1] >= 0 && !fenc.lowMvs[d0].empty() && (d1 == 0 || !fenc.lowMvs1[d1].empty()))
    {
        score = fenc.cost2[d0][d1] = fenc.specCost2[d0][d1];
        {
            const int key = d0 * 32 + d1;
            auto it = fenc.dSpecLc.find(key);
            if (it != fenc.dSpecLc.end()) { fenc.dropLc(fenc.dLc, key); fenc.dLc[key] = it->second; fenc.dSpecLc.erase(it); fenc.lcHost.erase(key); }
        }
        if (d1 == 0) { fenc.costEst[d0] = score; fenc.intraMbs[d0] = fenc.specIntraMbs[d0]; }
        return X265AMD_OK;
    }
    std::vector<CostJob> one(1);
    one[0].fenc = &fenc; one[0].ref0 = &ref0; one[0].ref1 = ref1; one[0].d0 = d0; one[0].d1 = d1;
    const int rc = frameCostMany(one);
    score = fenc.cost2[d0][d1];
    return rc;
}

void x265amd_encoder::laFieldPut(const void* key, void* mv, void* mc)
{
    auto it = laFields.find(key);
    if (it != laFields.end()) { laBufPut(it->second.mv); laBufPut(it->second.mc); it->second = DevField{ mv, mc, ++laFieldClock }; }
    else laFields.emplace(key, DevField{ mv, mc, ++laFieldClock });
}
void x265amd_encoder::laFieldsTrim()
{
    {
        std::vector<const void*> dead;
        { std::lock_guard<std::mutex> lk(laPool->mu); dead.swap(laPool->deadFields); }
        for (const void* k : dead)
        {
            auto it = laFields.find(k);
            if (it != laFields.end()) { laBufPut(it->second.mv); laBufPut(it->second.mc); laFields.erase(it); }
        }
    }
    if (laFields.size() <= LA_FIELDS_MAX) return;
    std::vector<uint64_t> ages;
    for (auto& f : laFields) ages.push_back(f.second.used);
    std::nth_element(ages.begin(), ages.begin() + ages.size() / 4, ages.end());
    const uint64_t cut = ages[ages.size() / 4];
    for (auto it = laFields.begin(); it != laFields.end();)
        if (it->second.used < cut) { laBufPut(it->second.mv); laBufPut(it->second.mc); it = laFields.erase(it); } else ++it;
}
void x265amd_encoder::laFieldsFree()
{
    for (auto& f : laFields) { laBufPut(f.second.mv); laBufPut(f.second.mc); }
    laFields.clear();
}

int x265amd_encoder::frameCostMany(std::vector<CostJob>& jobs)
{
    if (jobs.empty()) return X265AMD_OK;
    laFieldsTrim();
    const size_t ncu = (size_t)lowCuW * lowCuH;
    int rc = X265AMD_OK;
    const auto tb0 = std::chrono::steady_clock::now();
    struct Tm { x265amd_encoder* e; std::chrono::steady_clock::time_point t0; size_t n; ~Tm() { const double ms = std::chrono::duration<double, std::milli>(std::chrono::steady_clock::now() - t0).count(); if (n > 1) { e->laBatchMs += ms; e->laBatches++; } else { e->laSingleMs += ms; e->laSingles++; } } } tm_{ this, tb0, jobs.size() };
    std::vector<x265amd_lowres_cost_job> kj(jobs.size());
    size_t issued = 0;
    auto shared = [&](const std::vector<int16_t>& mv, const std::vector<int32_t>& mc, void*& dMv, void*& dMc) -> bool {
        auto it = laFields.find(mv.data());
        if (it == laFields.end())
        {
            void* a = laBuf(); void* b = laBuf();
            if (!a || !b) { laBufPut(a); laBufPut(b); return false; }
            laFieldPut(mv.data(), a, b);
            it = laFields.find(mv.data());
            if (hipMemcpyAsync(a, mv.data(), ncu * 4, hipMemcpyHostToDevice, laStream) != hipSuccess || hipMemcpyAsync(b, mc.data(), ncu * 4, hipMemcpyHostToDevice, laStream) != hipSuccess)
            { laBufPut(a); laBufPut(b); laFields.erase(mv.data()); return false; }
        }
        it->second.used = ++laFieldClock;
        dMv = it->second.mv; dMc = it->second.mc;
        return true;
    };
    auto tph = std::chrono::steady_clock::now();
    auto phase = [&](int i) { const auto t = std::chrono::steady_clock::now(); laPhaseMs[i] += std::chrono::duration<double, std::milli>(t - tph).count(); tph = t; };
    std::vector<LaWeight> lw(jobs.size());
    std::vector<int> wAt(jobs.size(), -1);
    std::vector<x265amd_weight_cost_job> wj;
    for (size_t k = 0; k < jobs.size(); k++)
    {
        CostJob& j = jobs[k];
        Pic& fenc = *j.fenc;
        if (!j.spec && (!j.whole || laNumSlices <= 1))
        {
            if (fenc.lowMvs[j.d0].empty() && !fenc.specMvs[j.d0].empty()) { fenc.lowMvs[j.d0].swap(fenc.specMvs[j.d0]); fenc.lowMvc[j.d0].swap(fenc.specMvc[j.d0]); }
            if (j.d1 > 0 && fenc.lowMvs1[j.d1].empty() && !fenc.specMvs1[j.d1].empty()) { fenc.lowMvs1[j.d1].swap(fenc.specMvs1[j.d1]); fenc.lowMvc1[j.d1].swap(fenc.specMvc1[j.d1]); }
        }
        const bool have0 = !fenc.lowMvs[j.d0].empty() || (j.spec && !fenc.specMvs[j.d0].empty()), have1 = j.d1 > 0 && (!fenc.lowMvs1[j.d1].empty() || (j.spec && !fenc.specMvs1[j.d1].empty()));
        j.search0 = !have0; j.search1 = j.d1 > 0 && !have1;
        static const char* const dbgWp = xa_env_str("X265AMD_WP_DEBUG");
        if (p.bEnableWeightedPred && j.search0 && !(dbgWp && strchr(dbgWp, 'l')) && lookaheadWeightGuess(fenc, *j.ref0, lw[k]))
        {
            x265amd_weight_cost_job w;
            memset(&w, 0, sizeof(w));
            w.d_fenc = fenc.dLowres + lowOrg; w.d_intra_cost = fenc.dIntraCost;
            for (int t = 0; t < 4; t++) w.d_ref[t] = j.ref0->dLowres + (size_t)t * lowPlaneElems + lowOrg;
            w.cands[1] = weightCand(lw[k].curScale, lw[k].mindenom, lw[k].curOffset);
            wAt[k] = (int)wj.size();
            wj.push_back(w);
        }
        laJobs++; laSearches += (j.search0 ? 1 : 0) + (j.search1 ? 1 : 0);
    }
    std::vector<uint32_t> wCosts(2 * wj.size() + 2);
    laWeightJobs += wj.size();
    if (!wj.empty()) rc = x265amd_lowres_weight_costs_many(laStream, wj.data(), (int)wj.size(), lowStride, lowW, lowH, wCosts.data());
    for (size_t k = 0; k < jobs.size() && rc == X265AMD_OK; k++)
    {
        CostJob& j = jobs[k];
        Pic& fenc = *j.fenc;
        bool weighted = false; int wScale = 0, wDenom = 0, wOffset = 0;
        if (wAt[k] >= 0) lookaheadWeightDecide(lw[k], &wCosts[2 * wAt[k]], weighted, wScale, wDenom, wOffset);
        void** bufs[6] = { &j.dLc, &j.dBc, &j.dMvs, &j.dMvc, &j.dMvs1, &j.dMvc1 };
        const size_t sizes[6] = { ncu * 2, ncu * 4, ncu * 4, ncu * 4, ncu * 4, ncu * 4 };
        const bool want[6] = { true, true, j.search0, j.search0, j.search1, j.search1 };
        (void)sizes;
        for (int b = 0; b < 6; b++) if (want[b] && !(*bufs[b] = laBuf())) rc = xa_fail(X265AMD_EHIP, "encoder: device allocation");
        issued = k + 1;
        if (rc != X265AMD_OK) break;
        x265amd_lowres_cost_job& q = kj[k];
        memset(&q, 0, sizeof(q));
        q.d_fenc = fenc.dLowres + lowOrg;
        for (int t = 0; t < 4; t++) { q.d_ref0[t] = j.ref0->dLowres + (size_t)t * lowPlaneElems + lowOrg; q.d_ref1[t] = j.ref1 ? j.ref1->dLowres + (size_t)t * lowPlaneElems + lowOrg : nullptr; }
        q.d_intra_cost = fenc.dIntraCost;
        q.d_lowres_costs = (uint16_t*)j.dLc; q.d_bcost = (int32_t*)j.dBc; q.do_search0 = j.search0; q.do_search1 = j.search1;
        if (!j.whole && laNumSlices > 1) { q.rows_per_slice = laRowsPerSlice; q.num_slices = laNumSlices; }
        if (weighted)
        {
            const int correction = 14 - X265AMD_DEPTH;
            if (xa_scratch_alloc(&j.dW, lowPlaneElems * 4 * sizeof(pixel)) != hipSuccess) { rc = xa_fail(X265AMD_EHIP, "encoder: device allocation"); break; }
            rc = x265amd_weight_buffer(laStream, j.ref0->dLowres, (pixel*)j.dW, lowPlaneElems * 4, wScale, (wDenom ? 1 << (wDenom - 1) : 0) << correction, wDenom + correction, wOffset << (X265AMD_DEPTH - 8));
            if (rc != X265AMD_OK) break;
            for (int t = 0; t < 4; t++) q.d_ref0w[t] = (pixel*)j.dW + (size_t)t * lowPlaneElems + lowOrg;
        }
        bool ok = true;
        const bool own0 = !fenc.lowMvs[j.d0].empty(), own1 = j.d1 > 0 && !fenc.lowMvs1[j.d1].empty();
        void* f0 = j.dMvs; void* c0 = j.dMvc; void* f1 = j.dMvs1; void* c1 = j.dMvc1;
        if (!j.search0) ok = shared((own0 ? fenc.lowMvs : fenc.specMvs)[j.d0], (own0 ? fenc.lowMvc : fenc.specMvc)[j.d0], f0, c0);
        if (ok && j.d1 > 0 && !j.search1) ok = shared((own1 ? fenc.lowMvs1 : fenc.specMvs1)[j.d1], (own1 ? fenc.lowMvc1 : fenc.specMvc1)[j.d1], f1, c1);
        q.d_mvs0 = (int16_t*)f0; q.d_mv_costs0 = (int32_t*)c0; q.d_mvs1 = (int16_t*)f1; q.d_mv_costs1 = (int32_t*)c1;
        if (!ok) rc = xa_fail(X265AMD_EHIP, "encoder: lowres frame cost set-up");
    }
    phase(0);
    if (rc == X265AMD_OK) rc = x265amd_lowres_frame_cost_batch(laStream, me, kj.data(), (int)jobs.size(), lowStride, lowCuW, lowCuH);
    std::vector<int64_t> sums(2 * jobs.size());
    if (rc == X265AMD_OK) rc = x265amd_lowres_cost_sums(laStream, kj.data(), (int)issued, lowCuW, lowCuH, sums.data());
    phase(1);
    for (size_t k = 0; k < issued && rc == X265AMD_OK; k++)
    {
        CostJob& j = jobs[k];
        Pic& fenc = *j.fenc;
        bool ok = true;
        if (ok && j.search0)
        {
            std::vector<int16_t>& mv = (j.spec ? fenc.specMvs : fenc.lowMvs)[j.d0]; std::vector<int32_t>& mc = (j.spec ? fenc.specMvc : fenc.lowMvc)[j.d0];
            mv.resize(ncu * 2); mc.resize(ncu);
            ok = hipMemcpyAsync(mv.data(), j.dMvs, ncu * 4, hipMemcpyDeviceToHost, laStream) == hipSuccess && hipMemcpyAsync(mc.data(), j.dMvc, ncu * 4, hipMemcpyDeviceToHost, laStream) == hipSuccess;
            if (ok) { laFieldPut(mv.data(), j.dMvs, j.dMvc); j.dMvs = j.dMvc = nullptr; }
        }
        if (ok && j.search1)
        {
            std::vector<int16_t>& mv = (j.spec ? fenc.specMvs1 : fenc.lowMvs1)[j.d1]; std::vector<int32_t>& mc = (j.spec ? fenc.specMvc1 : fenc.lowMvc1)[j.d1];
            mv.resize(ncu * 2); mc.resize(ncu);
            ok = hipMemcpyAsync(mv.data(), j.dMvs1, ncu * 4, hipMemcpyDeviceToHost, laStream) == hipSuccess && hipMemcpyAsync(mc.data(), j.dMvc1, ncu * 4, hipMemcpyDeviceToHost, laStream) == hipSuccess;
            if (ok) { laFieldPut(mv.data(), j.dMvs1, j.dMvc1); j.dMvs1 = j.dMvc1 = nullptr; }
        }
        if (!ok) rc = xa_fail(X265AMD_EHIP, "encoder: lowres frame cost");
    }
    phase(2);
    if (hipStreamSynchronize(laStream) != hipSuccess && rc == X265AMD_OK) rc = xa_fail(X265AMD_EHIP, "encoder: lowres frame cost");
    phase(3);
    struct Ph { decltype(phase)& f; ~Ph() { f(4); } } ph_{ phase };
    laFieldsTrim();
    for (size_t k = 0; k < issued; k++)
    {
        CostJob& j = jobs[k];
        void* keepLc = rc != X265AMD_OK ? nullptr : (p.cuTree ? j.dLc : (rateCtl && j.d1 == 0 ? j.dBc : nullptr));
        void* bufs[6] = { j.dMvs, j.dMvc, keepLc == j.dLc ? nullptr : j.dLc, keepLc == j.dBc ? nullptr : j.dBc, j.dMvs1, j.dMvc1 };
        for (void* b : bufs) laBufPut(b);
        xa_scratch_free(j.dW);
        j.dMvs = j.dMvc = j.dLc = j.dBc = j.dMvs1 = j.dMvc1 = j.dW = nullptr;
        if (keepLc)
        {
            const int key = j.d0 * 32 + j.d1;
            std::map<int, void*>& m = j.spec ? j.fenc->dSpecLc : j.fenc->dLc;
            j.fenc->dropLc(m, key);
            m[key] = keepLc;
            if (!j.spec) j.fenc->lcHost.erase(key);
        }
        if (rc != X265AMD_OK)
        {
            if (j.search0) { (j.spec ? j.fenc->specMvs : j.fenc->lowMvs)[j.d0].clear(); (j.spec ? j.fenc->specMvc : j.fenc->lowMvc)[j.d0].clear(); }
            if (j.search1) { (j.spec ? j.fenc->specMvs1 : j.fenc->lowMvs1)[j.d1].clear(); (j.spec ? j.fenc->specMvc1 : j.fenc->lowMvc1)[j.d1].clear(); }
            continue;
        }
        int64_t est = sums[2 * k]; const int imb = (int)sums[2 * k + 1];
        if (j.d1 > 0) est = est * 100 / (130 + 0);
        if (j.spec) { j.fenc->specCost2[j.d0][j.d1] = est; if (j.d1 == 0) j.fenc->specIntraMbs[j.d0] = imb; continue; }
        if (j.search0) { j.fenc->specMvs[j.d0].clear(); j.fenc->specMvc[j.d0].clear(); for (int t = 0; t < 18; t++) { j.fenc->specCost2[j.d0][t] = -1; j.fenc->dropLc(j.fenc->dSpecLc, j.d0 * 32 + t); } }
        if (j.search1) { j.fenc->specMvs1[j.d1].clear(); j.fenc->specMvc1[j.d1].clear(); for (int t = 0; t < 18; t++) { j.fenc->specCost2[t][j.d1] = -1; j.fenc->dropLc(j.fenc->dSpecLc, t * 32 + j.d1); } }
        j.fenc->cost2[j.d0][j.d1] = est;
        if (j.d1 == 0) { j.fenc->costEst[j.d0] = est; j.fenc->intraMbs[j.d0] = imb; }
    }
    return rc;
}
int x265amd_encoder::frameCost(std::vector<Pic*>& frames, int p0, int p1, int b, int64_t& score)
{
    return frameCostAt(*frames[b], *frames[p0], p1 > b ? frames[p1] : nullptr, b - p0, p1 - b, score);
}

int64_t x265amd_encoder::planCost(std::vector<Pic*>& frames, const std::vector<uint8_t>& runs, int64_t limit, int& rc)
{
    int64_t total = 0;
    int anchor = 0;
    for (size_t g = 0; g < runs.size() && rc == X265AMD_OK; g++)
    {
        const int pPic = anchor + runs[g] + 1;
        int64_t c = 0;
        rc = frameCost(frames, anchor, pPic, pPic, c);
        total += c;
        if (total > limit) break;
        if (p.bBPyramid && runs[g] > 1)
        {
            const int middle = anchor + (pPic - anchor) / 2;
            if (rc == X265AMD_OK) { rc = frameCost(frames, anchor, pPic, middle, c); total += c; }
            for (int b = anchor + 1; b < middle && total < limit && rc == X265AMD_OK; b++) { rc = frameCost(frames, anchor, middle, b, c); total += c; }
            for (int b = middle + 1; b < pPic && total < limit && rc == X265AMD_OK; b++) { rc = frameCost(frames, middle, pPic, b, c); total += c; }
        }
        else
            for (int b = anchor + 1; b < pPic && total < limit && rc == X265AMD_OK; b++) { rc = frameCost(frames, anchor, pPic, b, c); total += c; }
        anchor = pPic;
    }
    return total;
}
void x265amd_encoder::extendPlans(std::vector<Pic*>& frames, int length, std::vector<std::vector<uint8_t> >& plans, int& rc)
{
    const int longest = std::min(p.bframes, length - 1);
    int64_t cheapest = 1LL << 62;
    std::vector<uint8_t> winner;
    for (int run = 0; run <= longest && rc == X265AMD_OK; run++)
    {
        std::vector<uint8_t> plan = plans[length - (run + 1)];
        plan.push_back((uint8_t)run);
        const int64_t cost = planCost(frames, plan, cheapest, rc);
        if (cost < cheapest) { cheapest = cost; winner.swap(plan); }
    }
    plans[length] = winner;
}

bool x265amd_encoder::scenecutInternal(std::vector<Pic*>& frames, int p0, int p1, bool real, int& rc)
{
    Pic* frame = frames[p1];
    if (rc == X265AMD_OK) rc = frameCostP(*frame, *frames[p0], p1 - p0);
    if (rc != X265AMD_OK) return false;
    const int64_t icost = frame->costEst[0], pcost = frame->costEst[p1 - p0];
    const int gopSize = (int)(((int64_t)frame->poc - lastKeyframe) % p.keyframeMax);
    const float threshMax = (float)(p.scenecutThreshold / 100.0);
    float threshMin = (float)(threshMax * 0.25);
    double bias = 5.0 / 100;
    if (real)
    {
        if (keyframeMin == p.keyframeMax) threshMin = threshMax;
        if (gopSize <= keyframeMin / 4) bias = threshMin / 4;
        else if (gopSize <= keyframeMin) bias = threshMin * gopSize / keyframeMin;
        else bias = threshMin + (threshMax - threshMin) * (gopSize - keyframeMin) / (p.keyframeMax - keyframeMin);
    }
    return pcost >= (1.0 - bias) * icost;
}

bool x265amd_encoder::scenecut(std::vector<Pic*>& frames, int p0, int p1, bool real, int numFrames, int& rc)
{
    if (real && p.bframes)
    {
        const int origmaxp1 = p0 + 1 + p.bframes, maxp1 = std::min(origmaxp1, numFrames);
        bool fluctuate = false, noScenecuts = false;
        int64_t avgSatdCost = 0;
        if (frames[p0]->costEst[p1 - p0] > -1) avgSatdCost = frames[p0]->costEst[p1 - p0];
        int cnt = 1;
        for (int cp1 = p1; cp1 <= maxp1; cp1++)
        {
            if (!scenecutInternal(frames, p0, cp1, false, rc))
            {
                for (int i = cp1; i > p0; i--) { frames[i]->bScenecut = false; noScenecuts = false; }
            }
            else if (scenecutInternal(frames, cp1 - 1, cp1, false, rc)) { frames[cp1]->bScenecut = true; noScenecuts = true; }
            if (rc != X265AMD_OK) return false;
            avgSatdCost += frames[cp1]->costEst[cp1 - p0];
            cnt++;
        }
        if (noScenecuts)
        {
            fluctuate = false;
            avgSatdCost /= cnt;
            for (int i = p1; i <= maxp1; i++)
            {
                const int64_t curCost = frames[i]->costEst[i - p0], prevCost = frames[i - 1]->costEst[i - 1 - p0];
                if (fabs((double)(curCost - avgSatdCost)) > 0.1 * avgSatdCost || fabs((double)(curCost - prevCost)) > 0.1 * prevCost)
                {
                    fluctuate = true;
                    if (!isSceneTransition && frames[i]->bScenecut)
                    {
                        isSceneTransition = true;
                        for (int j = i + 1; j <= maxp1; j++) frames[j]->bScenecut = false;
                        break;
                    }
                }
                frames[i]->bScenecut = false;
            }
        }
        if (!fluctuate && !noScenecuts) isSceneTransition = false;
    }
    if (!frames[p1]->bScenecut) return false;
    return scenecutInternal(frames, p0, p1, real, rc);
}

bool x265amd_encoder::histBasedScenecut(std::vector<Pic*>& frames, int p0, int p1, int numFrames)
{
    if (p.bframes)
    {
        const int maxp1 = std::min(p0 + 1 + p.bframes, numFrames);
        for (int cp1 = p0; cp1 < maxp1; cp1++)
        {
            if (frames[cp1 + 1]->bHistScenecutAnalyzed) continue;
            if (cp1 + 2 >= (int)frames.size()) continue;
            Pic* prev = frames[cp1]; Pic* cur = frames[cp1 + 1]; Pic* next = frames[cp1 + 2];
            cur->bHistScenecutAnalyzed = true;
            if (x265amd_hist_scene_change(prev->hist.get(), cur->hist.get(), next->hist.get(), W, H, &histState, nullptr) == 1) cur->bScenecut = true;
        }
    }
    return frames[p1]->bScenecut;
}

int x265amd_encoder::slicetypeAnalyse(std::vector<Pic*>& frames, bool bKeyframe)
{
    const int maxSearch = std::min(p.lookaheadDepth, 250);
    int framecnt = 0;
    for (; framecnt < maxSearch; framecnt++)
        if (framecnt + 1 >= (int)frames.size() || frames[framecnt + 1]->type != TYPE_AUTO) break;
    if (!framecnt) return p.cuTree ? runCuTree(frames, 0, bKeyframe) : X265AMD_OK;
    frames.resize((size_t)framecnt + 1);
    const int keyFrameLimit = (int)std::min<int64_t>((int64_t)p.keyframeMax + lastKeyframe - frames[0]->poc - 1, INT_MAX / 2), keyintLimit = keyFrameLimit;
    const int origNumFrames = std::min(framecnt, keyintLimit);
    int numFrames = origNumFrames;
    if (p.bOpenGOP && numFrames < framecnt) numFrames++;
    else if (numFrames == 0) { frames[1]->type = TYPE_I; return X265AMD_OK; }
    int rc = X265AMD_OK;
    if (p.bFrameAdaptive == 2 && p.bframes)
    {
        std::vector<CostJob> jobs;
        for (int b = 2; b < numFrames; b++)
            for (int i = 1; i <= p.bframes + 1; i++)
            {
                const int p0 = b - i;
                if (p0 < 0 || !frames[b]->lowMvs[i].empty()) continue;
                int p1 = b + i;
                if (p1 >= numFrames || !frames[b]->lowMvs1[i].empty()) p1 = b;
                if (frames[b]->cost2[i][p1 - b] >= 0) continue;
                CostJob j;
                j.fenc = frames[b]; j.ref0 = frames[p0]; j.ref1 = p1 > b ? frames[p1] : nullptr; j.d0 = i; j.d1 = p1 - b; j.whole = true;
                jobs.push_back(j);
            }
        if (frames[1]->lowMvs[1].empty()) { CostJob j; j.fenc = frames[1]; j.ref0 = frames[0]; j.d0 = 1; jobs.push_back(j); }
        auto hasL0 = [](const Pic* f, int d) { return !f->lowMvs[d].empty() || !f->specMvs[d].empty(); };
        auto hasL1 = [](const Pic* f, int d) { return !f->lowMvs1[d].empty() || !f->specMvs1[d].empty(); };
        for (int i = 1; i <= p.bframes + 1 && i <= numFrames && numFrames > 1; i++)
            if (!hasL0(frames[numFrames], i)) { CostJob j; j.fenc = frames[numFrames]; j.ref0 = frames[numFrames - i]; j.d0 = i; j.spec = true; jobs.push_back(j); }
        rc = frameCostMany(jobs);
        if (rc != X265AMD_OK) return rc;
        jobs.clear();
        for (int b = 1; b < numFrames; b++)
            for (int jj = 1; jj <= p.bframes; jj++)
            {
                const int p1 = b + jj;
                if (p1 > numFrames) break;
                if (hasL1(frames[b], jj) || !hasL0(frames[b], 1)) continue;
                CostJob j;
                j.fenc = frames[b]; j.ref0 = frames[b - 1]; j.ref1 = frames[p1]; j.d0 = 1; j.d1 = jj; j.spec = true;
                jobs.push_back(j);
            }
        rc = frameCostMany(jobs);
        if (rc != X265AMD_OK) return rc;
        jobs.clear();
        for (int b = 1; b < numFrames; b++)
            for (int i = 1; i <= p.bframes + 1; i++)
            {
                if (b < i || !hasL0(frames[b], i)) continue;
                for (int jj = 0; jj <= p.bframes; jj++)
                {
                    const int p1 = b + jj;
                    if (p1 > numFrames) break;
                    if ((jj && !hasL1(frames[b], jj)) || frames[b]->cost2[i][jj] >= 0 || frames[b]->specCost2[i][jj] >= 0) continue;
                    CostJob j;
                    j.fenc = frames[b]; j.ref0 = frames[b - i]; j.ref1 = jj ? frames[p1] : nullptr; j.d0 = i; j.d1 = jj;
                    j.spec = !(b >= 2 && p1 < numFrames && !frames[b]->lowMvs[i].empty() && (!jj || !frames[b]->lowMvs1[jj].empty()));
                    jobs.push_back(j);
                }
            }
        for (int i = 1; i <= p.bframes + 1 && i <= numFrames; i++)
            if (hasL0(frames[numFrames], i) && frames[numFrames]->cost2[i][0] < 0 && frames[numFrames]->specCost2[i][0] < 0)
            { CostJob j; j.fenc = frames[numFrames]; j.ref0 = frames[numFrames - i]; j.d0 = i; j.spec = true; jobs.push_back(j); }
        rc = frameCostMany(jobs);
        if (rc != X265AMD_OK) return rc;
    }
    const bool isScenecut = p.bHistBasedSceneCut ? histBasedScenecut(frames, 0, 1, origNumFrames) : scenecut(frames, 0, 1, true, origNumFrames, rc);
    if (rc != X265AMD_OK) return rc;
    if (p.scenecutThreshold > 0 && isScenecut) { frames[1]->type = TYPE_I; return X265AMD_OK; }
    int resetStart;
    if (p.bframes)
    {
        int numBFrames = std::min(numFrames - 1, p.bframes);
        if (p.bFrameAdaptive == 2)
        {
            numBFrames = 0;
            if (numFrames > 1)
            {
                std::vector<std::vector<uint8_t> > plans((size_t)numFrames + 1);
                plans[1].push_back(0);
                for (int j = 2; j <= numFrames && rc == X265AMD_OK; j++) extendPlans(frames, j, plans, rc);
                if (rc != X265AMD_OK) return rc;
                const std::vector<uint8_t>& plan = plans[numFrames];
                numBFrames = plan.empty() ? 0 : plan[0];
                int at = 1;
                for (size_t g = 0; g < plan.size(); g++)
                {
                    for (int k = 0; k < plan[g] && at < numFrames; k++) frames[at++]->type = TYPE_B;
                    if (at < numFrames) frames[at++]->type = TYPE_P;
                }
            }
        }
        else if (p.bFrameAdaptive == 1)
        {
            const int cuCount = lowBlocks;
            auto cost = [&](int p0, int p1, int b, bool intraPenalty, int64_t& out) -> int {
                int64_t sc = 0;
                const int r = frameCost(frames, p0, p1, b, sc);
                if (r != X265AMD_OK) return r;
                if (intraPenalty) sc += sc * frames[b]->intraMbs[b - p0] / (cuCount * 8);
                out = sc;
                return X265AMD_OK;
            };
            for (int i = 0; i <= numFrames - 2 && rc == X265AMD_OK; )
            {
                int64_t cost1p0 = 0, cost2p0 = 0, cost1b1 = 0, cost2p1 = 0;
                if ((rc = cost(i + 0, i + 2, i + 2, true, cost2p1)) != X265AMD_OK) break;
                if (frames[i + 2]->intraMbs[2] > cuCount / 2) { frames[i + 1]->type = TYPE_P; frames[i + 2]->type = TYPE_P; i += 2; continue; }
                if ((rc = cost(i + 0, i + 2, i + 1, false, cost1b1)) != X265AMD_OK || (rc = cost(i + 0, i + 1, i + 1, false, cost1p0)) != X265AMD_OK ||
                    (rc = cost(i + 1, i + 2, i + 2, false, cost2p0)) != X265AMD_OK) break;
                if (cost1p0 + cost2p0 < cost1b1 + cost2p1) { frames[i + 1]->type = TYPE_P; i += 1; continue; }
                frames[i + 1]->type = TYPE_B;
                int j;
                for (j = i + 2; j <= std::min(i + p.bframes, numFrames - 1); j++)
                {
                    const int64_t pthresh = std::max(300 - (50 - 0) * (j - i - 1), 300 / 10);
                    int64_t pcost = 0;
                    if ((rc = cost(i + 0, j + 1, j + 1, true, pcost)) != X265AMD_OK) break;
                    if (pcost > pthresh * cuCount || frames[j + 1]->intraMbs[j - i + 1] > cuCount / 3) break;
                    frames[j]->type = TYPE_B;
                }
                if (rc != X265AMD_OK) break;
                frames[j]->type = TYPE_P;
                i = j;
            }
            if (rc != X265AMD_OK) return rc;
            frames[numFrames]->type = TYPE_P;
            numBFrames = 0;
            while (numBFrames < numFrames && frames[numBFrames + 1]->type == TYPE_B) numBFrames++;
        }
        else
            for (int j = 1; j < numFrames; j++) frames[j]->type = (j % (numBFrames + 1)) ? TYPE_B : TYPE_P;
        frames[numFrames]->type = TYPE_P;
        int numAnalyzed = numFrames;
        for (int j = 1; j < numBFrames + 1; j++)
        {
            const bool cut = scenecut(frames, j, j + 1, false, origNumFrames, rc);
            if (rc != X265AMD_OK) return rc;
            if (cut) { frames[j]->type = TYPE_P; numAnalyzed = j; break; }
        }
        resetStart = bKeyframe ? 1 : std::min(numBFrames + 2, numAnalyzed + 1);
    }
    else
    {
        for (int j = 1; j <= numFrames; j++) frames[j]->type = TYPE_P;
        resetStart = bKeyframe ? 1 : 2;
    }
    if (p.cuTree && (rc = runCuTree(frames, std::min(numFrames, p.keyframeMax), bKeyframe)) != X265AMD_OK) return rc;
    for (int64_t j = (int64_t)keyintLimit + 1; j <= numFrames; j += p.keyframeMax) { frames[j]->type = TYPE_I; resetStart = std::min(resetStart, (int)j + 1); }
    const int maxp1 = std::min(p.bframes + 1, origNumFrames);
    for (int j = resetStart; j <= numFrames; j++)
    {
        frames[j]->type = TYPE_AUTO;
        if (j <= maxp1 && frames[j]->bScenecut && isSceneTransition) isSceneTransition = false;
    }
    return X265AMD_OK;
}

namespace { struct TreeCtx { x265amd_encoder* e; std::vector<Pic*>* frames; }; }
int x265amd_encoder::cuTreeEstimate(void* ctx, int p0, int p1, int b, const uint16_t** lc, const int16_t** mvs0, const int16_t** mvs1)
{
    TreeCtx& t = *(TreeCtx*)ctx;
    x265amd_encoder& e = *t.e;
    std::vector<Pic*>& frames = *t.frames;
    if (p0 < 0 || b < p0 || p1 < b || p1 >= (int)frames.size() || b - p0 > 17 || p1 - b > 17 || b == p0) return xa_fail(X265AMD_EINVAL, "encoder: cuTree estimate");
    int64_t score = 0;
    const int rc = e.frameCost(frames, p0, p1, b, score);
    if (rc != X265AMD_OK) return rc;
    Pic& f = *frames[b];
    const int d0 = b - p0, d1 = p1 - b, key = d0 * 32 + d1;
    auto h = f.lcHost.find(key);
    if (h == f.lcHost.end())
    {
        auto d = f.dLc.find(key);
        if (d == f.dLc.end()) return xa_fail(X265AMD_EHIP, "encoder: cuTree: the block costs of an estimate are gone");
        std::vector<uint16_t> v((size_t)e.lowCuW * e.lowCuH);
        if (hipMemcpyAsync(v.data(), d->second, v.size() * 2, hipMemcpyDeviceToHost, e.laStream) != hipSuccess || hipStreamSynchronize(e.laStream) != hipSuccess)
            return xa_fail(X265AMD_EHIP, "encoder: cuTree: block costs");
        h = f.lcHost.emplace(key, std::move(v)).first;
    }
    *lc = h->second.data();
    *mvs0 = f.lowMvs[d0].empty() ? nullptr : f.lowMvs[d0].data();
    *mvs1 = d1 > 0 && !f.lowMvs1[d1].empty() ? f.lowMvs1[d1].data() : nullptr;
    return 0;
}
int x265amd_encoder::runCuTree(std::vector<Pic*>& frames, int numframes, bool bIntra)
{
    if (numframes >= (int)frames.size()) numframes = (int)frames.size() - 1;
    std::vector<x265amd_cutree_frame> recs(frames.size());
    std::vector<x265amd_cutree_frame*> ptrs(frames.size());
    for (size_t k = 0; k < frames.size(); k++)
    {
        Pic& f = *frames[k];
        if (f.intraCostHost.empty() || f.qpAqOffset.empty()) return xa_fail(X265AMD_EINVAL, "encoder: cuTree: a picture without block offsets");
        x265amd_cutree_frame& r = recs[k];
        memset(&r, 0, sizeof(r));
        r.slice_type = f.type; r.intra_cost = f.intraCostHost.data(); r.inv_qscale = f.invQscale.data(); r.qp_aq_offset = f.qpAqOffset.data();
        r.qp_cutree_offset = f.qpCuTreeOffset.data(); r.propagate_cost = f.propagateCost.data(); r.weighted_cost_delta = nullptr;
        ptrs[k] = &r;
    }
    TreeCtx ctx{ this, &frames };
    const int rc = x265amd_cutree(&treeParams, ptrs.data(), numframes, bIntra, cuTreeEstimate, &ctx);
    return rc == X265AMD_OK ? X265AMD_OK : xa_fail(rc, "encoder: cuTree");
}

void x265amd_encoder::pushMiniGop(int b)
{
    if (p.bBPyramid && b > 1) input[b / 2]->type = TYPE_BREF;
    if (b > 0) input[b - 1]->bLastMiniGopBFrame = true;
    ready.push_back(input[b]);
    for (int i = 0; i < b; i++) if (input[i]->type == TYPE_BREF) ready.push_back(input[i]);
    for (int i = 0; i < b; i++) if (input[i]->type != TYPE_BREF) ready.push_back(input[i]);
    input.erase(input.begin(), input.begin() + b + 1);
    first = false;
}

int x265amd_encoder::decideLookahead(bool flush, int maxGops)
{
    const int fullQueue = flush ? 1 : std::max(1, p.lookaheadDepth);
    while ((int)input.size() >= fullQueue && maxGops-- > 0)
    {
        const int maxSearch = std::max(1, std::min(p.lookaheadDepth, 250));
        std::vector<Pic*> frames;
        frames.push_back(lastNonB.get());
        for (int j = 0; j < maxSearch && j < (int)input.size(); j++) frames.push_back(input[j].get());
        const int windowCount = (int)frames.size() - 1;
        if (lastNonB)
        {
            const int rc = slicetypeAnalyse(frames);
            if (rc != X265AMD_OK) return rc;
        }
        const int nlist = std::min((int)input.size(), p.bframes + 2);
        int b = 0;
        for (;; b++)
        {
            Pic& frm = *input[b];
            if ((int64_t)frm.poc - lastKeyframe >= p.keyframeMax && (frm.type == TYPE_AUTO || frm.type == TYPE_I)) frm.type = p.bOpenGOP && haveKeyframe ? TYPE_I : TYPE_IDR;
            if (frm.type == TYPE_I && (int64_t)frm.poc - lastKeyframe >= keyframeMin)
            {
                if (p.bOpenGOP) { lastKeyframe = frm.poc; frm.bKeyframe = true; haveKeyframe = true; }
                else frm.type = TYPE_IDR;
            }
            if (frm.type == TYPE_IDR)
            {
                lastKeyframe = frm.poc; frm.bKeyframe = true; haveKeyframe = true;
                if (b > 0) { input[b - 1]->type = TYPE_P; b--; }
            }
            Pic& cur = *input[b];
            if (&cur == &frm)
            {
                if (b == p.bframes || b + 1 >= nlist) { if (frm.type == TYPE_AUTO || frm.type == TYPE_B) frm.type = TYPE_P; }
                if (frm.type == TYPE_AUTO) frm.type = TYPE_B;
                else if (frm.type != TYPE_B) break;
            }
            else break;
        }
        if (p.rateControlMode == X265AMD_RC_CRF)
        {
            if (p.bBPyramid && b > 1) input[b / 2]->type = TYPE_BREF;
            std::vector<Pic*> est;
            est.push_back(lastNonB.get());
            for (int i = 0; i <= b; i++) est.push_back(input[i].get());
            int64_t score = 0;
            const int p1n = b + 1;
            const bool isI = est[p1n]->type == TYPE_I || est[p1n]->type == TYPE_IDR;
            if (!isI && est[0])
            {
                const int rc = frameCost(est, 0, p1n, p1n, score);
                if (rc != X265AMD_OK) return rc;
            }
            if (b && est[0])
            {
                int p0 = 0;
                bool isp0available = est[p1n]->type != TYPE_IDR;
                for (int bb = 1; bb <= b; bb++)
                {
                    if (!isp0available) p0 = bb;
                    int p1;
                    if (est[bb]->type == TYPE_B) for (p1 = bb; est[p1]->type == TYPE_B; p1++) { }
                    else p1 = b + 1;
                    if (p0 != bb)
                    {
                        const int rc = frameCost(est, p0, p1, bb, score);
                        if (rc != X265AMD_OK) return rc;
                    }
                    if (est[bb]->type == TYPE_BREF) { p0 = bb; isp0available = true; }
                }
            }
        }
        lastNonB = input[b];
        pushMiniGop(b);
        if (p.cuTree && (lastNonB->type == TYPE_I || lastNonB->type == TYPE_IDR))
        {
            std::vector<Pic*> kf;
            kf.push_back(lastNonB.get());
            const int left = windowCount - (b + 1);
            for (int j = 0; j < left && j < (int)input.size(); j++) kf.push_back(input[j].get());
            const int rc = slicetypeAnalyse(kf, true);
            if (rc != X265AMD_OK) return rc;
        }
    }
    return X265AMD_OK;
}

void x265amd_encoder::decideMiniGop(bool flush)
{
    while (!input.empty())
    {
        if (!flush && (int)input.size() < p.bframes + 1 && !(first && !input.empty())) return;
        int b = 0;
        for (;; b++)
        {
            Pic& frm = *input[b];
            if ((int64_t)frm.poc - lastKeyframe >= p.keyframeMax) frm.type = p.bOpenGOP && haveKeyframe ? TYPE_I : TYPE_IDR;
            if (frm.type == TYPE_I)
            {
                lastKeyframe = frm.poc; frm.bKeyframe = true;
                break;
            }
            if (frm.type == TYPE_IDR)
            {
                if (b > 0) { input[b - 1]->type = TYPE_P; b--; break; }
                lastKeyframe = frm.poc; frm.bKeyframe = true; haveKeyframe = true;
                break;
            }
            if (b == p.bframes || b + 1 >= (int)input.size()) { frm.type = TYPE_P; break; }
            frm.type = TYPE_B;
        }
        pushMiniGop(b);
        if (!flush) return;
    }
}
```

### x265-amod_amd/csrc/plane_kernels.hip

```cpp
#include "x265amd_dev.h"
#include "x265amd_host.h"

__global__ __launch_bounds__(256) void k_extend_border(pixel* pic, long stride, int width, int height, int marginX, int marginY, int firstRow)
{
    const int y = firstRow + (int)blockIdx.x;
    const int cy = min(max(y, 0), height - 1);
    const pixel* srcRow = pic + (long)cy * stride;
    pixel* dstRow = pic + (long)y * stride;
    if (y >= 0 && y < height)
    {
        const pixel l = srcRow[0], r = srcRow[width - 1];
        for (int i = threadIdx.x; i < 2 * marginX; i += blockDim.x)
        {
            if (i < marginX) dstRow[-marginX + i] = l;
            else dstRow[width + (i - marginX)] = r;
        }
        return;
    }
    for (int x = -marginX + (int)threadIdx.x; x < width + marginX; x += blockDim.x)
        dstRow[x] = srcRow[min(max(x, 0), width - 1)];
}

__global__ __launch_bounds__(256) void k_extend_band(pixel* pic, long stride, int width, int height, int marginX, int marginY, int y0, int y1, int xa, int xb, int doLeft, int doRight)
{
    int y = y0 + (int)blockIdx.x;
    const int bottomLines = y1 == height ? marginY : 0;
    if (y >= y1 + bottomLines) y = -1 - (y - y1 - bottomLines);
    if (y >= 0 && y < y1)
    {
        pixel* row = pic + (long)y * stride;
        const pixel l = row[0], r = row[width - 1];
        for (int i = threadIdx.x; i < marginX; i += blockDim.x)
        {
            if (doLeft) row[-marginX + i] = l;
            if (doRight) row[width + i] = r;
        }
        return;
    }
    const pixel* src = pic + (long)(y < 0 ? 0 : height - 1) * stride;
    pixel* dst = pic + (long)y * stride;
    const int from = (doLeft && xa == 0) ? -marginX : xa, to = (doRight && xb == width) ? width + marginX : xb;
    for (int x = from + (int)threadIdx.x; x < to; x += blockDim.x) dst[x] = src[min(max(x, 0), width - 1)];
}

struct ExtendBand3 { pixel* pic[3]; long stride[3]; int width[3], height[3], marginX[3], marginY[3], y0[3], y1[3], xa[3], xb[3]; int doLeft, doRight; };
__global__ __launch_bounds__(256) void k_extend_band3(ExtendBand3 E)
{
    const int p = blockIdx.y;
    pixel* pic = E.pic[p];
    const long stride = E.stride[p];
    const int width = E.width[p], height = E.height[p], marginX = E.marginX[p], marginY = E.marginY[p], y0 = E.y0[p], y1 = E.y1[p], xa = E.xa[p], xb = E.xb[p];
    const int lines = (y1 - y0) + (y1 == height ? marginY : 0) + (y0 == 0 ? marginY : 0);
    if ((int)blockIdx.x >= lines) return;
    int y = y0 + (int)blockIdx.x;
    const int bottomLines = y1 == height ? marginY : 0;
    if (y >= y1 + bottomLines) y = -1 - (y - y1 - bottomLines);
    if (y >= 0 && y < y1)
    {
        pixel* row = pic + (long)y * stride;
        const pixel l = row[0], r = row[width - 1];
        for (int i = threadIdx.x; i < marginX; i += blockDim.x)
        {
            if (E.doLeft) row[-marginX + i] = l;
            if (E.doRight) row[width + i] = r;
        }
        return;
    }
    const pixel* src = pic + (long)(y < 0 ? 0 : height - 1) * stride;
    pixel* dst = pic + (long)y * stride;
    const int from = (E.doLeft && xa == 0) ? -marginX : xa, to = (E.doRight && xb == width) ? width + marginX : xb;
    for (int x = from + (int)threadIdx.x; x < to; x += blockDim.x) dst[x] = src[min(max(x, 0), width - 1)];
}

__global__ __launch_bounds__(256) void k_weight_plane(const pixel* src, pixel* dst, long stride, int width, int height, int marginX, int marginY,
                                                      int w0, int round, int shift, int offset)
{
    const int y = (int)blockIdx.x - marginY;
    const int cy = min(max(y, 0), height - 1);
    const pixel* srcRow = src + (long)cy * stride;
    pixel* dstRow = dst + (long)y * stride;
    const int correction = XA_IF_INTERNAL_PREC - XA_DEPTH;
    for (int x = -marginX + (int)threadIdx.x; x < width + marginX; x += blockDim.x)
    {
        const int v = (int)srcRow[min(max(x, 0), width - 1)] << correction;
        dstRow[x] = xa_clip_pixel(((w0 * v + round) >> shift) + offset);
    }
}

extern "C" int x265amd_extend_pic_border(void* stream, x265amd_pixel* d_pic, intptr_t stride, int width, int height, int marginX, int marginY)
{
    return x265amd_extend_border_rows(stream, d_pic, stride, width, height, marginX, marginY, 0, height);
}

extern "C" int x265amd_extend_border_rows(void* stream, x265amd_pixel* d_pic, intptr_t stride, int width, int height, int marginX, int marginY, int y_begin, int y_end)
{
    if (!d_pic || width <= 0 || height <= 0 || marginX < 0 || marginY < 0 || y_begin < 0 || y_begin >= y_end || y_end > height)
        return xa_fail(X265AMD_EINVAL, "x265amd_extend_pic_border: bad arguments");
    const int first = y_begin == 0 ? -marginY : y_begin, last = y_end == height ? height + marginY : y_end;
    hipLaunchKernelGGL(k_extend_border, dim3(last - first), dim3(256), 0, (hipStream_t)stream, (pixel*)d_pic, (long)stride, width, height, marginX, marginY, first);
    hipError_t e = hipGetLastError();
    if (e != hipSuccess) return xa_fail(X265AMD_EHIP, hipGetErrorString(e));
    return X265AMD_OK;
}

extern "C" int x265amd_extend_border_band(void* stream, x265amd_pixel* d_pic, intptr_t stride, int width, int height, int marginX, int marginY, int y_begin, int y_end,
                                          int x_begin, int x_end, int left, int right)
{
    if (!d_pic || width <= 0 || height <= 0 || marginX < 0 || marginY < 0 || y_begin < 0 || y_begin >= y_end || y_end > height || x_begin < 0 || x_begin >= x_end || x_end > width)
        return xa_fail(X265AMD_EINVAL, "x265amd_extend_border_band: bad arguments");
    const int lines = (y_end - y_begin) + (y_end == height ? marginY : 0) + (y_begin == 0 ? marginY : 0);
    hipLaunchKernelGGL(k_extend_band, dim3(lines), dim3(256), 0, (hipStream_t)stream, (pixel*)d_pic, (long)stride, width, height, marginX, marginY, y_begin, y_end, x_begin, x_end,
                       left, right);
    hipError_t e = hipGetLastError();
    if (e != hipSuccess) return xa_fail(X265AMD_EHIP, hipGetErrorString(e));
    return X265AMD_OK;
}

int xa_extend_border_band_420(void* stream, x265amd_pixel* d_y, x265amd_pixel* d_u, x265amd_pixel* d_v, intptr_t stride, intptr_t cstride, int width, int height, int marginX, int marginY,
                              int y_begin, int y_end, int x_begin, int x_end, int left, int right)
{
    if (!d_y || !d_u || !d_v || width <= 0 || height <= 0 || marginX < 0 || marginY < 0 || y_begin < 0 || y_begin >= y_end || y_end > height || x_begin < 0 || x_begin >= x_end || x_end > width ||
        ((width | height | marginX | marginY | y_begin | y_end | x_begin | x_end) & 1))
        return xa_fail(X265AMD_EINVAL, "xa_extend_border_band_420: bad arguments");
    ExtendBand3 E;
    for (int p = 0; p < 3; p++)
    {
        const int sh = p ? 1 : 0;
        E.pic[p] = (pixel*)(p == 0 ? d_y : (p == 1 ? d_u : d_v)); E.stride[p] = (long)(p ? cstride : stride);
        E.width[p] = width >> sh; E.height[p] = height >> sh; E.marginX[p] = marginX >> sh; E.marginY[p] = marginY >> sh;
        E.y0[p] = y_begin >> sh; E.y1[p] = y_end >> sh; E.xa[p] = x_begin >> sh; E.xb[p] = x_end >> sh;
    }
    E.doLeft = left; E.doRight = right;
    const int lines = (y_end - y_begin) + (y_end == height ? marginY : 0) + (y_begin == 0 ? marginY : 0);
    hipLaunchKernelGGL(k_extend_band3, dim3(lines, 3), dim3(256), 0, (hipStream_t)stream, E);
    hipError_t e = hipGetLastError();
    if (e != hipSuccess) return xa_fail(X265AMD_EHIP, hipGetErrorString(e));
    return X265AMD_OK;
}

extern "C" int x265amd_extend_border_band_420(void* stream, x265amd_pixel* d_y, x265amd_pixel* d_u, x265amd_pixel* d_v, intptr_t stride, intptr_t cstride, int width, int height,
                                              int marginX, int marginY, int y_begin, int y_end, int x_begin, int x_end, int left, int right)
{
    return xa_extend_border_band_420(stream, d_y, d_u, d_v, stride, cstride, width, height, marginX, marginY, y_begin, y_end, x_begin, x_end, left, right);
}

extern "C" int x265amd_weight_plane(void* stream, const x265amd_pixel* d_src, x265amd_pixel* d_dst, intptr_t stride, int width, int height,
                                    int marginX, int marginY, int inputWeight, int inputOffset, int log2WeightDenom)
{
    if (!d_src || !d_dst || width <= 0 || height <= 0 || marginX < 0 || marginY < 0) return xa_fail(X265AMD_EINVAL, "x265amd_weight_plane: bad arguments");
    const int correction = XA_IF_INTERNAL_PREC - XA_DEPTH;
    const int offset = inputOffset * (1 << (XA_DEPTH - 8));
    const int round = (log2WeightDenom ? 1 << (log2WeightDenom - 1) : 0) << correction;
    hipLaunchKernelGGL(k_weight_plane, dim3(height + 2 * marginY), dim3(256), 0, (hipStream_t)stream, (const pixel*)d_src, (pixel*)d_dst, (long)stride,
                       width, height, marginX, marginY, inputWeight, round, log2WeightDenom + correction, offset);
    hipError_t e = hipGetLastError();
    if (e != hipSuccess) return xa_fail(X265AMD_EHIP, hipGetErrorString(e));
    return X265AMD_OK;
}
```

Measured before the change: 104.8.

## Overlap picture upload, buffer clears and lowres read-back with encoding via async streams

Picture upload moves to a dedicated non-blocking stream. The recon and final-buffer memsets no longer block: events record when the source is ready and when all buffers are ready, and frame tasks and row imports wait on the ready event. The device-input path replaces per-plane 2D copies plus border-extension launches with one fused kernel that copies and pads all three planes. Lookahead lowres host read-back is deferred to a finisher thread, with guards that abort if results are read early. This trades default-stream serialization for more events, a thread and more complex ordering.

```diff
diff --git a/x265-amod_amd/csrc/encoder_api.hip b/x265-amod_amd/csrc/encoder_api.hip
--- a/x265-amod_amd/csrc/encoder_api.hip
+++ b/x265-amod_amd/csrc/encoder_api.hip
@@ -380,6 +380,7 @@
     if (in->map_offset_units + in->units_bytes > pic->units.size() * sizeof(x265amd_cu_unit) || in->map_offset_motion + in->motion_bytes > pic->motion.size() * sizeof(x265amd_mv_unit))
         return xa_fail(X265AMD_EINVAL, "encoder_import_row: map range"), -1;
     xa_thread_device();
+    if (pic->waitReady()) { pic->fail(); return xa_fail(X265AMD_EHIP, "encoder_import_row: the picture's buffers"), -1; }
     uint8_t* dst = (uint8_t*)(pic->dFin ? pic->dFin : pic->dRec);
     {
         std::lock_guard<std::mutex> lk(e->importMu);
@@ -426,30 +427,34 @@
 
 int x265amd_encoder::uploadPicture(const x265amd_picture* in, Pic& pic, bool onDevice)
 {
+    if (!upStream && hipStreamCreateWithFlags(&upStream, hipStreamNonBlocking) != hipSuccess) { upStream = nullptr; return xa_fail(X265AMD_EHIP, "encoder_encode: stream"); }
+    for (int k = 0; k < 3; k++)
+        if (!in->planes[k] || in->stride[k] < (int)((k ? srcW / 2 : srcW) * sizeof(pixel))) return xa_fail(X265AMD_EINVAL, "encoder_encode: input plane");
+    if (xa_scratch_alloc((void**)&pic.dSrc, picElems * sizeof(pixel)) != hipSuccess || xa_scratch_alloc((void**)&pic.dRec, picElems * sizeof(pixel)) != hipSuccess ||
+        (frameParallel && p.bEnableSAO && xa_scratch_alloc((void**)&pic.dFin, picElems * sizeof(pixel)) != hipSuccess))
+        return xa_fail(X265AMD_EHIP, "encoder_encode: device allocation");
+    if (hipEventCreateWithFlags(&pic.evSrc, hipEventDisableTiming) != hipSuccess || hipEventCreateWithFlags(&pic.evReady, hipEventDisableTiming) != hipSuccess)
+        return xa_fail(X265AMD_EHIP, "encoder_encode: event");
+    auto finish = [&](int rc, const char* what) -> int {
+        const bool a = hipEventRecord(pic.evSrc, upStream) == hipSuccess;
+        const bool b = hipMemsetAsync(pic.dRec, 0, picElems * sizeof(pixel), upStream) == hipSuccess && (!pic.dFin || hipMemsetAsync(pic.dFin, 0, picElems * sizeof(pixel), upStream) == hipSuccess);
+        const bool c = hipEventRecord(pic.evReady, upStream) == hipSuccess;
+        if (rc) return rc;
+        if (!a || !b || !c) return xa_fail(X265AMD_EHIP, "encoder_encode: memset");
+        return hipEventSynchronize(pic.evSrc) == hipSuccess ? 0 : xa_fail(X265AMD_EHIP, what);
+    };
     if (onDevice)
     {
-        if (xa_scratch_alloc((void**)&pic.dSrc, picElems * sizeof(pixel)) != hipSuccess || xa_scratch_alloc((void**)&pic.dRec, picElems * sizeof(pixel)) != hipSuccess)
-            return xa_fail(X265AMD_EHIP, "encoder_encode: device allocation");
-        if (hipMemsetAsync(pic.dSrc, 0, picElems * sizeof(pixel), nullptr) != hipSuccess) return xa_fail(X265AMD_EHIP, "encoder_encode: memset");
+        const void* const src[3] = { in->planes[0], in->planes[1], in->planes[2] };
+        const int srcStride[3] = { in->stride[0], in->stride[1], in->stride[2] };
         for (int k = 0; k < 3; k++)
         {
-            const int w = k ? W / 2 : W, h = k ? H / 2 : H, mx = k ? marginX / 2 : marginX, my = k ? marginY / 2 : marginY;
-            const intptr_t st = k ? cstride : stride;
-            const int sw = k ? srcW / 2 : srcW, sh = k ? srcH / 2 : srcH;
-            if (!in->planes[k] || in->stride[k] < (int)(sw * sizeof(pixel))) return xa_fail(X265AMD_EINVAL, "encoder_encode: input plane");
-            if (hipMemcpy2DAsync(pic.dSrc + org[k], (size_t)st * sizeof(pixel), in->planes[k], (size_t)in->stride[k], (size_t)sw * sizeof(pixel), (size_t)sh, hipMemcpyDeviceToDevice, nullptr) != hipSuccess)
-                return xa_fail(X265AMD_EHIP, "encoder_encode: the input picture is not device memory of this device");
-            if ((sw != w || sh != h) && x265amd_extend_pic_border(nullptr, (x265amd_pixel*)(pic.dSrc + org[k]), st, sw, sh, w - sw, h - sh) != X265AMD_OK) return -1;
-            if (x265amd_extend_pic_border(nullptr, (x265amd_pixel*)(pic.dSrc + org[k]), st, w, h, mx, my) != X265AMD_OK) return -1;
-        }
-        if (hipMemsetAsync(pic.dRec, 0, picElems * sizeof(pixel), nullptr) != hipSuccess) return xa_fail(X265AMD_EHIP, "encoder_encode: memset");
-        if (frameParallel && p.bEnableSAO)
-        {
-            if (xa_scratch_alloc((void**)&pic.dFin, picElems * sizeof(pixel)) != hipSuccess) return xa_fail(X265AMD_EHIP, "encoder_encode: device allocation");
-            if (hipMemsetAsync(pic.dFin, 0, picElems * sizeof(pixel), nullptr) != hipSuccess) return xa_fail(X265AMD_EHIP, "encoder_encode: memset");
-        }
-        if (hipStreamSynchronize(nullptr) != hipSuccess) return xa_fail(X265AMD_EHIP, "encoder_encode: the input picture's copy");
-        return 0;
+            hipPointerAttribute_t attr;
+            if (hipPointerGetAttributes(&attr, src[k]) != hipSuccess || (attr.type != hipMemoryTypeDevice && attr.type != hipMemoryTypeManaged))
+            { (void)hipGetLastError(); return finish(xa_fail(X265AMD_EHIP, "encoder_encode: the input picture is not device memory of this device"), ""); }
+        }
+        const int rc = xa_input_picture_420(upStream, (x265amd_pixel*)pic.dSrc, org, picElems, stride, cstride, W, H, marginX, marginY, src, srcStride, srcW, srcH);
+        return finish(rc == X265AMD_OK ? 0 : -1, "encoder_encode: the input picture is not device memory of this device");
     }
     if (!uploadBuf)
     {
@@ -461,7 +466,6 @@
         const int w = k ? W / 2 : W, h = k ? H / 2 : H, mx = k ? marginX / 2 : marginX, my = k ? marginY / 2 : marginY;
         const intptr_t st = k ? cstride : stride;
         const int sw = k ? srcW / 2 : srcW, sh = k ? srcH / 2 : srcH;
-        if (!in->planes[k] || in->stride[k] < (int)(sw * sizeof(pixel))) return xa_fail(X265AMD_EINVAL, "encoder_encode: input plane");
         pixel* base = uploadBuf + org[k];
         for (int y = 0; y < h; y++)
         {
@@ -477,16 +481,8 @@
             memcpy(base + (intptr_t)(h - 1 + y) * st - mx, base + (intptr_t)(h - 1) * st - mx, sizeof(pixel) * (w + 2 * mx));
         }
     }
-    if (xa_scratch_alloc((void**)&pic.dSrc, picElems * sizeof(pixel)) != hipSuccess || xa_scratch_alloc((void**)&pic.dRec, picElems * sizeof(pixel)) != hipSuccess)
-        return xa_fail(X265AMD_EHIP, "encoder_encode: device allocation");
-    if (hipMemcpy(pic.dSrc, uploadBuf, picElems * sizeof(pixel), hipMemcpyHostToDevice) != hipSuccess) return xa_fail(X265AMD_EHIP, "encoder_encode: upload");
-    if (hipMemset(pic.dRec, 0, picElems * sizeof(pixel)) != hipSuccess || hipStreamSynchronize(nullptr) != hipSuccess) return xa_fail(X265AMD_EHIP, "encoder_encode: memset");
-    if (frameParallel && p.bEnableSAO)
-    {
-        if (xa_scratch_alloc((void**)&pic.dFin, picElems * sizeof(pixel)) != hipSuccess) return xa_fail(X265AMD_EHIP, "encoder_encode: device allocation");
-        if (hipMemset(pic.dFin, 0, picElems * sizeof(pixel)) != hipSuccess || hipStreamSynchronize(nullptr) != hipSuccess) return xa_fail(X265AMD_EHIP, "encoder_encode: memset");
-    }
-    return 0;
+    const bool sent = hipMemcpyAsync(pic.dSrc, uploadBuf, picElems * sizeof(pixel), hipMemcpyHostToDevice, upStream) == hipSuccess;
+    return finish(sent ? 0 : xa_fail(X265AMD_EHIP, "encoder_encode: upload"), "encoder_encode: upload");
 }
 
 static int encoder_encode_impl(x265amd_encoder* e, x265amd_nal** ppNal, uint32_t* piNal, const x265amd_picture* picIn, x265amd_picture* picOut, bool inputOnDevice);
@@ -509,11 +505,13 @@
         pic->pool = e->laPool;
         pic->poc = e->frameCount++;
         const auto tu0 = std::chrono::steady_clock::now();
+        if (e->firstInMs < 0) e->firstInMs = Pic::pubClockMs();
         int rc = e->uploadPicture(picIn, *pic, inputOnDevice);
         if (rc) return -1;
         const auto tl0 = std::chrono::steady_clock::now();
         e->uploadMs += std::chrono::duration<double, std::milli>(tl0 - tu0).count();
         if (e->lookahead && (rc = e->lowresInit(*pic)) != X265AMD_OK) return -1;
+        if (e->lookahead) e->lowresFinishLater(pic);
         e->laInitMs += std::chrono::duration<double, std::milli>(std::chrono::steady_clock::now() - tl0).count();
         e->input.push_back(pic);
     }
@@ -548,9 +546,15 @@
         std::shared_future<int> prev = e->lastTask;
         pic->started = true;
         if (timing) fprintf(stderr, "x265amd: poc %d handed to a frame task at %.1f ms (%d running)\n", pic->poc, Pic::pubClockMs(), e->running);
+        if (timing && !e->startReported && e->firstInMs >= 0)
+        {
+            e->startReported = true;
+            fprintf(stderr, "x265amd: start-up: %.1f ms from the first picture handed in to the first frame task (poc %d)\n", Pic::pubClockMs() - e->firstInMs, pic->poc);
+        }
         pic->done = std::async(std::launch::async, [e, pic, prev, timing]() {
             xa_thread_device();
             const auto t0 = std::chrono::steady_clock::now();
+            if (pic->waitReady()) { pic->fail(); return xa_fail(X265AMD_EHIP, "encoder: the picture's buffers"); }
             if (!pic->owned)
             {
                 if (pic->type == TYPE_B) { if (!e->keepSources()) { xa_scratch_free(pic->dSrc); pic->dSrc = nullptr; } return (int)X265AMD_OK; }
diff --git a/x265-amod_amd/csrc/encoder_impl.h b/x265-amod_amd/csrc/encoder_impl.h
--- a/x265-amod_amd/csrc/encoder_impl.h
+++ b/x265-amod_amd/csrc/encoder_impl.h
@@ -24,6 +24,9 @@
 #include <memory>
 #include <vector>
 
+int xa_input_picture_420(void* stream, x265amd_pixel* d_pic, const size_t org[3], size_t pic_elems, intptr_t stride, intptr_t cstride, int width, int height, int marginX, int marginY,
+                         const void* const src[3], const int src_stride_bytes[3], int src_width, int src_height);
+
 namespace xaenc {
 
 typedef x265amd_pixel pixel;
@@ -67,6 +70,14 @@
     int importedRows = 0;
     bool hasReferences = false;
     pixel* dSrc = nullptr; pixel* dRec = nullptr;
+    hipEvent_t evSrc = nullptr, evReady = nullptr;
+    int waitReady() { return !evReady || hipEventSynchronize(evReady) == hipSuccess ? 0 : -1; }
+    hipEvent_t evLowres = nullptr;
+    void* laStage = nullptr;
+    std::atomic<bool> lowresPending{ false };
+    std::mutex lowresMu;
+    int lowresRc = 0;
+    void needLowres() const { if (lowresPending.load(std::memory_order_acquire)) { fprintf(stderr, "x265amd: fatal: a picture's lowres results are read before lowresFinish (poc %d)\n", poc); abort(); } }
     std::vector<x265amd_cu_unit> units;
     std::vector<x265amd_mv_unit> motion;
     int32_t refPoc[2][16];
@@ -121,7 +132,8 @@
         if (!xa_devmap_register(regMotion, motion.size())) regMotion = nullptr;
     }
     Pic() { memset(refPoc, 0, sizeof(refPoc)); memset(wp, 0, sizeof(wp)); for (int i = 0; i < 18; i++) { costEst[i] = -1; intraMbs[i] = 0; specIntraMbs[i] = 0; for (int j = 0; j < 18; j++) cost2[i][j] = specCost2[i][j] = -1; } }
-    ~Pic() { if (pool) { for (auto& e : dLc) pool->put(e.second); for (auto& e : dSpecLc) pool->put(e.second);
+    ~Pic() { for (hipEvent_t ev : { evSrc, evReady, evLowres }) if (ev) { (void)hipEventSynchronize(ev); (void)hipEventDestroy(ev); } if (laStage) xa_mapped_free(laStage);
+             if (pool) { for (auto& e : dLc) pool->put(e.second); for (auto& e : dSpecLc) pool->put(e.second);
                          for (int i = 0; i < 18; i++) for (const std::vector<int16_t>* v : { &lowMvs[i], &lowMvs1[i], &specMvs[i], &specMvs1[i] }) if (!v->empty()) pool->dead(v->data()); } if (regMotion) xa_devmap_unregister(regMotion); xa_scratch_free(dSrc); xa_scratch_free(dRec); xa_scratch_free(dFin); xa_scratch_free(dLowres); xa_scratch_free(dIntraCost); if (edgeCounts) xa_mapped_free(edgeCounts); for (volatile uint64_t* c : finalX) xa_counter_free(c); }
     void publish(int row, int x)
     {
@@ -173,6 +185,7 @@
     std::shared_future<int> lastTask;
     int frameThreads = 1;
     double uploadMs = 0;
+    double firstInMs = -1; bool startReported = false;
     std::atomic<uint64_t> cpuPictureNs{ 0 }, cpuFilterNs{ 0 };
     bool frameParallel = false;
     int refLagRows = 0;
@@ -182,12 +195,19 @@
     std::vector<x265amd_nal> nals;
     std::vector<pixel> staging;
     pixel* uploadBuf = nullptr;
+    hipStream_t upStream = nullptr;
     int32_t* dSaoCount = nullptr; int32_t* dSaoOrg = nullptr; x265amd_sao_ctu* dSaoParams = nullptr; x265amd_deblock_unit* dDbUnits = nullptr;
     pixel* dSaoTmp = nullptr;
 
     ~x265amd_encoder()
     {
         for (auto& q : inflight) if (q->done.valid()) q->done.wait();
+        if (laFinisher.joinable())
+        {
+            { std::lock_guard<std::mutex> lk(laFinMu); laFinStop = true; }
+            laFinCv.notify_all();
+            laFinisher.join();
+        }
         laFieldsFree();
         if (uploadBuf) (void)hipHostFree(uploadBuf);
         if (xa_env_present("X265AMD_TIMING") && lookahead)
@@ -196,6 +216,8 @@
             fprintf(stderr, "x265amd: lookahead: %.1f ms in lowres planes + intra costs, %.1f ms in the slice-type decision (%llu estimates, %llu motion searches; %llu batches %.1f ms, %llu single estimates %.1f ms)\n", laInitMs, laDecideMs,
                     (unsigned long long)laJobs, (unsigned long long)laSearches, (unsigned long long)laBatches, laBatchMs, (unsigned long long)laSingles, laSingleMs);
             fprintf(stderr, "x265amd: lookahead estimates by phase: set-up %.1f ms, launch call %.1f, read-back issued %.1f, waited for %.1f, host sums %.1f; %llu weight guesses measured\n", laPhaseMs[0], laPhaseMs[1], laPhaseMs[2], laPhaseMs[3], laPhaseMs[4], (unsigned long long)laWeightJobs);
+            fprintf(stderr, "x265amd: slice-type analysis by part: batch searches %.1f ms, fields left to the trellis %.1f, costs %.1f, scene cut + trellis %.1f, cuTree %.1f; host arithmetic behind the lowres wait %.1f\n",
+                    laAnalyseMs[0], laAnalyseMs[1], laAnalyseMs[2], laAnalyseMs[3], laAnalyseMs[4], laFinishNs.load() / 1e6);
         }
         if (me) x265amd_me_close(me);
         if (rateCtl) x265amd_rc_close(rateCtl);
@@ -205,7 +227,8 @@
         if (dDbUnits) (void)hipFree(dDbUnits);
         xa_scratch_free(dSaoTmp);
         xa_scratch_free(histRecord);
-        if (histRecordHost) xa_mapped_free(histRecordHost);
+        if (upStream) { (void)hipStreamSynchronize(upStream); (void)hipStreamDestroy(upStream); }
+        if (laStream) (void)hipStreamSynchronize(laStream);
         if (laStream) (void)hipStreamDestroy(laStream);
         if (importStream) (void)hipStreamDestroy(importStream);
     }
@@ -219,7 +242,7 @@
     int runFrameParallel(const PicP& pic);
     int edgeCounts(Pic& pic, hipStream_t st, x265amd_rskip_edge& edge);
     bool lookahead = false;
-    void* wpEnergy = nullptr; void* wpSums = nullptr; void* wpSumsHost = nullptr; void* wpMvs = nullptr;
+    void* wpEnergy = nullptr; void* wpSums = nullptr; void* wpMvs = nullptr;
     int laRowsPerSlice = 0, laNumSlices = 1;
     int keyframeMin = 1, lowW = 0, lowH = 0, lowCuW = 0, lowCuH = 0, lowBlocks = 0;
     intptr_t lowStride = 0; size_t lowPlaneElems = 0, lowOrg = 0;
@@ -227,6 +250,11 @@
     bool isSceneTransition = false;
     hipStream_t laStream = nullptr;
     int lowresInit(Pic& pic);
+    int lowresFinish(Pic& pic);
+    std::thread laFinisher; std::mutex laFinMu; std::condition_variable laFinCv; std::deque<PicP> laFinQueue; bool laFinStop = false;
+    void lowresFinishLater(const PicP& pic);
+    std::atomic<uint64_t> laFinishNs{ 0 };
+    size_t laStageBytes() const;
     void pushMiniGop(int b);
     struct LaWeight { int minscale = 0, mindenom = 0, curScale = 0, curOffset = 0; };
     bool lookaheadWeightGuess(Pic& fenc, Pic& ref, LaWeight& g);
@@ -250,13 +278,14 @@
     void laFieldsTrim();
     void laFieldsFree();
     double laPhaseMs[5] = { 0, 0, 0, 0, 0 };
+    double laAnalyseMs[5] = { 0, 0, 0, 0, 0 };
     double laInitMs = 0, laDecideMs = 0, laBatchMs = 0, laSingleMs = 0; uint64_t laJobs = 0, laSearches = 0, laBatches = 0, laSingles = 0, laWeightJobs = 0;
     int frameCost(std::vector<Pic*>& frames, int p0, int p1, int b, int64_t& score);
     int64_t planCost(std::vector<Pic*>& frames, const std::vector<uint8_t>& runs, int64_t limit, int& rc);
     void extendPlans(std::vector<Pic*>& frames, int length, std::vector<std::vector<uint8_t> >& plans, int& rc);
     bool scenecutInternal(std::vector<Pic*>& frames, int p0, int p1, bool real, int& rc);
     bool scenecut(std::vector<Pic*>& frames, int p0, int p1, bool real, int numFrames, int& rc);
-    void* histRecord = nullptr; void* histRecordHost = nullptr;
+    void* histRecord = nullptr;
     x265amd_hist_scene_state histState;
     bool histBasedScenecut(std::vector<Pic*>& frames, int p0, int p1, int numFrames);
     int slicetypeAnalyse(std::vector<Pic*>& frames, bool bKeyframe = false);
@@ -264,7 +293,7 @@
     x265amd_rc* rateCtl = nullptr;
     bool useDqp = false; int maxCuDqpDepth = 0;
     bool aqOn = false;
-    void* aqEnergy = nullptr; void* aqEnergyHost = nullptr; void* aqSums = nullptr;
+    void* aqEnergy = nullptr; void* aqSums = nullptr;
     x265amd_cutree_params treeParams;
     int adaptiveQuant(Pic& pic);
     int runCuTree(std::vector<Pic*>& frames, int numframes, bool bIntra);
diff --git a/x265-amod_amd/csrc/encoder_lookahead.hip b/x265-amod_amd/csrc/encoder_lookahead.hip
--- a/x265-amod_amd/csrc/encoder_lookahead.hip
+++ b/x265-amod_amd/csrc/encoder_lookahead.hip
@@ -1,9 +1,31 @@
 #include "encoder_impl.h"
 
+namespace {
+struct LaStageAt { size_t sums, density, intra, hist, total; };
+inline LaStageAt laStageAt(const x265amd_encoder& e)
+{
+    auto up = [](size_t v) { return (v + 63) & ~(size_t)63; };
+    const size_t nb = (size_t)((e.W + 15) / 16) * ((e.H + 15) / 16), ncu = (size_t)e.lowCuW * e.lowCuH;
+    LaStageAt a;
+    a.sums = up(nb * 4); a.density = up(a.sums + 6 * 8); a.intra = up(a.density + nb * 8); a.hist = up(a.intra + ncu * 4);
+    a.total = a.hist + (e.p.bHistBasedSceneCut ? X265AMD_HIST_SCENE_RECORD_BYTES(e.H) : 0);
+    return a;
+}
+}
+size_t x265amd_encoder::laStageBytes() const { return laStageAt(*this).total; }
+
 int x265amd_encoder::lowresInit(Pic& pic)
 {
-    if (xa_scratch_alloc((void**)&pic.dLowres, lowPlaneElems * 4 * sizeof(pixel)) != hipSuccess || xa_scratch_alloc((void**)&pic.dIntraCost, (size_t)lowCuW * lowCuH * 4 + (size_t)lowCuW * lowCuH) != hipSuccess)
+    const LaStageAt at = laStageAt(*this);
+    char* stage = nullptr;
+    if (xa_scratch_alloc((void**)&pic.dLowres, lowPlaneElems * 4 * sizeof(pixel)) != hipSuccess || xa_scratch_alloc((void**)&pic.dIntraCost, (size_t)lowCuW * lowCuH * 4 + (size_t)lowCuW * lowCuH) != hipSuccess ||
+        xa_mapped_alloc(&pic.laStage, at.total, true) != hipSuccess)
         return xa_fail(X265AMD_EHIP, "encoder_encode: device allocation");
+    stage = (char*)pic.laStage;
+    if (hipEventCreateWithFlags(&pic.evLowres, hipEventDisableTiming) != hipSuccess) return xa_fail(X265AMD_EHIP, "encoder_encode: event");
+    if (pic.evSrc && hipStreamWaitEvent(laStream, pic.evSrc, 0) != hipSuccess) return xa_fail(X265AMD_EHIP, "encoder_encode: event");
+    pic.lowresPending = true;
+    struct Rec { hipEvent_t ev; hipStream_t st; ~Rec() { (void)hipEventRecord(ev, st); } } rec_{ pic.evLowres, laStream };
     if (hipMemsetAsync(pic.dLowres, 0, lowPlaneElems * 4 * sizeof(pixel), laStream) != hipSuccess) return xa_fail(X265AMD_EHIP, "encoder_encode: memset");
     pixel* planes[4];
     for (int k = 0; k < 4; k++) planes[k] = pic.dLowres + (size_t)k * lowPlaneElems + lowOrg;
@@ -18,32 +40,68 @@
     if (sums && !aqOn)
     {
         const int bw = (W + 15) / 16, bh = (H + 15) / 16;
-        if (!wpEnergy && (xa_scratch_alloc(&wpEnergy, (size_t)bw * bh * 4) != hipSuccess || xa_scratch_alloc(&wpSums, 6 * 8) != hipSuccess || xa_mapped_alloc(&wpSumsHost, 6 * 8, true) != hipSuccess ||
+        if (!wpEnergy && (xa_scratch_alloc(&wpEnergy, (size_t)bw * bh * 4) != hipSuccess || xa_scratch_alloc(&wpSums, 6 * 8) != hipSuccess ||
                           xa_mapped_alloc(&wpMvs, (size_t)lowCuW * lowCuH * 4, false) != hipSuccess))
             return xa_fail(X265AMD_EHIP, "encoder_encode: device allocation");
         const uint64_t srcP[3] = { planeAddr(pic.dSrc, 0), planeAddr(pic.dSrc, 1), planeAddr(pic.dSrc, 2) };
         rc = x265amd_aq_energy(laStream, srcP, stride, cstride, W, H, 16, (uint32_t*)wpEnergy, (uint64_t*)wpSums);
-        if (rc == X265AMD_OK && hipMemcpyAsync(wpSumsHost, wpSums, 6 * 8, hipMemcpyDeviceToHost, laStream) != hipSuccess) rc = xa_fail(X265AMD_EHIP, "encoder_encode: picture sums");
+        if (rc == X265AMD_OK && hipMemcpyAsync(stage + at.sums, wpSums, 6 * 8, hipMemcpyDeviceToHost, laStream) != hipSuccess) rc = xa_fail(X265AMD_EHIP, "encoder_encode: picture sums");
         if (rc != X265AMD_OK) return rc;
     }
     if (aqOn && (rc = adaptiveQuant(pic)) != X265AMD_OK) return rc;
     if (p.bHistBasedSceneCut)
     {
         const size_t bytes = X265AMD_HIST_SCENE_RECORD_BYTES(H);
-        if (!histRecord && (xa_scratch_alloc(&histRecord, bytes) != hipSuccess || xa_mapped_alloc(&histRecordHost, bytes, true) != hipSuccess))
-            return xa_fail(X265AMD_EHIP, "encoder_encode: device allocation");
+        if (!histRecord && xa_scratch_alloc(&histRecord, bytes) != hipSuccess) return xa_fail(X265AMD_EHIP, "encoder_encode: device allocation");
         const uint64_t srcP[3] = { planeAddr(pic.dSrc, 0), planeAddr(pic.dSrc, 1), planeAddr(pic.dSrc, 2) };
         rc = x265amd_hist_scene_stats(laStream, srcP, stride, cstride, (uint64_t)(uintptr_t)planes[0], lowStride, W, H, (x265amd_hist_scene_record*)histRecord, 0);
         if (rc != X265AMD_OK) return rc;
-        if (hipMemcpyAsync(histRecordHost, histRecord, bytes, hipMemcpyDeviceToHost, laStream) != hipSuccess) return xa_fail(X265AMD_EHIP, "encoder_encode: picture statistics");
-    }
-    std::vector<int32_t> ic((size_t)lowCuW * lowCuH);
-    if (hipMemcpyAsync(ic.data(), pic.dIntraCost, ic.size() * 4, hipMemcpyDeviceToHost, laStream) != hipSuccess || hipStreamSynchronize(laStream) != hipSuccess)
-        return xa_fail(X265AMD_EHIP, "encoder_encode: lowres intra costs");
+        if (hipMemcpyAsync(stage + at.hist, histRecord, bytes, hipMemcpyDeviceToHost, laStream) != hipSuccess) return xa_fail(X265AMD_EHIP, "encoder_encode: picture statistics");
+    }
+    if (hipMemcpyAsync(stage + at.intra, pic.dIntraCost, (size_t)lowCuW * lowCuH * 4, hipMemcpyDeviceToHost, laStream) != hipSuccess) return xa_fail(X265AMD_EHIP, "encoder_encode: lowres intra costs");
+    return X265AMD_OK;
+}
+
+void x265amd_encoder::lowresFinishLater(const PicP& pic)
+{
+    if (!laFinisher.joinable())
+        laFinisher = std::thread([this]() {
+            xa_thread_device();
+            for (;;)
+            {
+                PicP pic;
+                {
+                    std::unique_lock<std::mutex> lk(laFinMu);
+                    laFinCv.wait(lk, [this] { return laFinStop || !laFinQueue.empty(); });
+                    if (laFinStop) return;
+                    pic = laFinQueue.front(); laFinQueue.pop_front();
+                }
+                (void)lowresFinish(*pic);
+            }
+        });
+    { std::lock_guard<std::mutex> lk(laFinMu); laFinQueue.push_back(pic); }
+    laFinCv.notify_one();
+}
+
+int x265amd_encoder::lowresFinish(Pic& pic)
+{
+    std::lock_guard<std::mutex> once(pic.lowresMu);
+    if (!pic.lowresPending.load(std::memory_order_acquire)) return pic.lowresRc ? xa_fail(pic.lowresRc, "encoder_encode: a picture's lowres results") : X265AMD_OK;
+    struct Done { Pic& pic; int& rc; ~Done() { pic.lowresRc = rc; pic.lowresPending.store(false, std::memory_order_release); } };
+    int rc = X265AMD_EHIP;
+    Done done_{ pic, rc };
+    if (!pic.evLowres || !pic.laStage || hipEventSynchronize(pic.evLowres) != hipSuccess) return xa_fail(X265AMD_EHIP, "encoder_encode: lowres intra costs");
+    rc = X265AMD_OK;
+    const auto tf0 = std::chrono::steady_clock::now();
+    struct Tf { std::atomic<uint64_t>& ns; std::chrono::steady_clock::time_point t0; ~Tf() { ns += (uint64_t)std::chrono::duration_cast<std::chrono::nanoseconds>(std::chrono::steady_clock::now() - t0).count(); } } tf_{ laFinishNs, tf0 };
+    const LaStageAt at = laStageAt(*this);
+    const char* stage = (const char*)pic.laStage;
+    const int32_t* ic = (const int32_t*)(stage + at.intra);
+    const size_t ncu = (size_t)lowCuW * lowCuH;
     if (p.bHistBasedSceneCut)
     {
         pic.hist.reset(new x265amd_hist_scene_pic);
-        if (x265amd_hist_scene_finish((const x265amd_hist_scene_record*)histRecordHost, W, H, pic.hist.get()) != X265AMD_OK) return xa_fail(X265AMD_EINVAL, "encoder_encode: picture statistics");
+        if (x265amd_hist_scene_finish((const x265amd_hist_scene_record*)(stage + at.hist), W, H, pic.hist.get()) != X265AMD_OK) return rc = xa_fail(X265AMD_EINVAL, "encoder_encode: picture statistics");
         pic.bHistScenecutAnalyzed = false;
     }
     if (aqOn)
@@ -52,14 +110,14 @@
         pic.qpAqOffset.assign((size_t)nb, 0.0); pic.qpCuTreeOffset.assign((size_t)nb, 0.0); pic.invQscale.assign((size_t)nb, 256);
         if (p.aqStrength != 0 && p.aqMode >= 4)
         {
-            const uint32_t* density = (const uint32_t*)((const char*)aqEnergyHost + (size_t)nb * 4 + 6 * 8);
-            rc = x265amd_aq_offsets_edge((const uint32_t*)aqEnergyHost, density, density + nb, nb, lowCuW * lowCuH, p.aqMode, p.aqStrength, 1.0, 16, pic.qpAqOffset.data(), pic.qpCuTreeOffset.data(), pic.invQscale.data());
+            const uint32_t* density = (const uint32_t*)(stage + at.density);
+            rc = x265amd_aq_offsets_edge((const uint32_t*)stage, density, density + nb, nb, lowCuW * lowCuH, p.aqMode, p.aqStrength, 1.0, 16, pic.qpAqOffset.data(), pic.qpCuTreeOffset.data(), pic.invQscale.data());
         }
         else if (p.aqStrength != 0)
-            rc = x265amd_aq_offsets((const uint32_t*)aqEnergyHost, nb, lowCuW * lowCuH, p.aqMode, p.aqStrength, 1.0, 16, pic.qpAqOffset.data(), pic.qpCuTreeOffset.data(), pic.invQscale.data());
-        if (rc != X265AMD_OK) return xa_fail(rc, "encoder_encode: adaptive quantisation");
-        pic.intraCostHost = ic;
-        if (p.cuTree) pic.propagateCost.assign((size_t)lowCuW * lowCuH, 0);
+            rc = x265amd_aq_offsets((const uint32_t*)stage, nb, lowCuW * lowCuH, p.aqMode, p.aqStrength, 1.0, 16, pic.qpAqOffset.data(), pic.qpCuTreeOffset.data(), pic.invQscale.data());
+        if (rc != X265AMD_OK) return rc = xa_fail(rc, "encoder_encode: adaptive quantisation");
+        pic.intraCostHost.assign(ic, ic + ncu);
+        if (p.cuTree) pic.propagateCost.assign(ncu, 0);
     }
     int64_t est = 0;
     const bool all = lowCuW <= 2 || lowCuH <= 2;
@@ -67,10 +125,11 @@
         for (int x = 0; x < lowCuW; x++)
             if (all || (x > 0 && x < lowCuW - 1 && y > 0 && y < lowCuH - 1)) est += ic[(size_t)y * lowCuW + x];
     pic.costEst[0] = est;
-    if (sums)
+    static const char* const dbgWp = xa_env_str("X265AMD_WP_DEBUG");
+    if ((p.bEnableWeightedPred || p.bEnableWeightedBiPred) && !(dbgWp && strchr(dbgWp, 's')))
     {
         uint64_t wp[6];
-        memcpy(wp, aqOn ? (const void*)((const char*)aqEnergyHost + (size_t)((W + 15) / 16) * ((H + 15) / 16) * 4) : wpSumsHost, sizeof(wp));
+        memcpy(wp, stage + at.sums, sizeof(wp));
         const int maxCol = ((W + 8) >> 4) << 4, maxRow = ((H + 8) >> 4) << 4;
         const int width[3] = { maxCol, maxCol >> 1, maxCol >> 1 }, height[3] = { maxRow, maxRow >> 1, maxRow >> 1 };
         for (int i = 0; i < 3; i++)
@@ -80,6 +139,7 @@
             pic.wpSsd[i] = ssd - (sum * sum + (uint64_t)((width[i] * height[i]) / 2)) / (uint64_t)(width[i] * height[i]);
         }
     }
+    xa_mapped_free(pic.laStage); pic.laStage = nullptr;
     return X265AMD_OK;
 }
 
@@ -87,9 +147,11 @@
 {
     const int bw = (W + 15) / 16, bh = (H + 15) / 16;
     const size_t nb = (size_t)bw * bh;
+    const LaStageAt at = laStageAt(*this);
+    char* stage = (char*)pic.laStage;
     const bool edge = p.aqMode >= 4 && p.aqStrength != 0;
     const size_t perBlock = edge ? 12 : 4;
-    if (!aqEnergy && (xa_scratch_alloc(&aqEnergy, nb * perBlock) != hipSuccess || xa_scratch_alloc(&aqSums, 6 * 8) != hipSuccess || xa_mapped_alloc(&aqEnergyHost, nb * perBlock + 6 * 8, true) != hipSuccess))
+    if (!aqEnergy && (xa_scratch_alloc(&aqEnergy, nb * perBlock) != hipSuccess || xa_scratch_alloc(&aqSums, 6 * 8) != hipSuccess))
         return xa_fail(X265AMD_EHIP, "encoder_encode: device allocation");
     if ((p.bEnableWeightedPred || p.bEnableWeightedBiPred) && !wpMvs && xa_mapped_alloc(&wpMvs, (size_t)lowCuW * lowCuH * 4, false) != hipSuccess)
         return xa_fail(X265AMD_EHIP, "encoder_encode: device allocation");
@@ -101,11 +163,11 @@
         uint32_t* density = (uint32_t*)aqEnergy + nb;
         rc = xa_aq_edge(laStream, srcP[0], stride, W, H, 16, density, density + nb, (uint64_t*)aqSums, (uint64_t*)aqSums + 3, 0, 0);
         if (rc != X265AMD_OK) return rc;
-        if (hipMemcpyAsync((char*)aqEnergyHost + nb * 4 + 6 * 8, density, nb * 8, hipMemcpyDeviceToHost, laStream) != hipSuccess)
+        if (hipMemcpyAsync(stage + at.density, density, nb * 8, hipMemcpyDeviceToHost, laStream) != hipSuccess)
             return xa_fail(X265AMD_EHIP, "encoder_encode: edge densities");
     }
-    if (hipMemcpyAsync(aqEnergyHost, aqEnergy, nb * 4, hipMemcpyDeviceToHost, laStream) != hipSuccess ||
-        hipMemcpyAsync((char*)aqEnergyHost + nb * 4, aqSums, 6 * 8, hipMemcpyDeviceToHost, laStream) != hipSuccess)
+    if (hipMemcpyAsync(stage, aqEnergy, nb * 4, hipMemcpyDeviceToHost, laStream) != hipSuccess ||
+        hipMemcpyAsync(stage + at.sums, aqSums, 6 * 8, hipMemcpyDeviceToHost, laStream) != hipSuccess)
         return xa_fail(X265AMD_EHIP, "encoder_encode: block energies");
     return X265AMD_OK;
 }
@@ -127,6 +189,7 @@
 {
     static const float epsilon = 1.f / 128.f;
     float guessScale, fencMean, refMean;
+    fenc.needLowres(); ref.needLowres();
     if (fenc.wpSsd[0] && ref.wpSsd[0]) guessScale = sqrtf((float)fenc.wpSsd[0] / ref.wpSsd[0]);
     else guessScale = 1.0f;
     fencMean = (float)fenc.wpSum[0] / (lowH * lowW) / (1 << (X265AMD_DEPTH - 8));
@@ -182,6 +245,7 @@
     {
         x265amd_weight* weights = pic.wp[list][0];
         Pic& ref = *pic.lists[list][0];
+        pic.needLowres(); ref.needLowres();
         const int diffPoc = abs(pic.poc - ref.poc);
         float guessScale[3], fencMean[3], refMean[3];
         for (int plane = 0; plane < 3; plane++)
@@ -669,6 +733,7 @@
 {
     const int maxSearch = std::min(p.lookaheadDepth, 250);
     int framecnt = 0;
+    for (const Pic* f : frames) if (f) f->needLowres();
     for (; framecnt < maxSearch; framecnt++)
         if (framecnt + 1 >= (int)frames.size() || frames[framecnt + 1]->type != TYPE_AUTO) break;
     if (!framecnt) return p.cuTree ? runCuTree(frames, 0, bKeyframe) : X265AMD_OK;
@@ -679,6 +744,8 @@
     if (p.bOpenGOP && numFrames < framecnt) numFrames++;
     else if (numFrames == 0) { frames[1]->type = TYPE_I; return X265AMD_OK; }
     int rc = X265AMD_OK;
+    auto tpa = std::chrono::steady_clock::now();
+    auto part = [&](int i) { const auto t = std::chrono::steady_clock::now(); laAnalyseMs[i] += std::chrono::duration<double, std::milli>(t - tpa).count(); tpa = t; };
     if (p.bFrameAdaptive == 2 && p.bframes)
     {
         std::vector<CostJob> jobs;
@@ -700,6 +767,7 @@
         for (int i = 1; i <= p.bframes + 1 && i <= numFrames && numFrames > 1; i++)
             if (!hasL0(frames[numFrames], i)) { CostJob j; j.fenc = frames[numFrames]; j.ref0 = frames[numFrames - i]; j.d0 = i; j.spec = true; jobs.push_back(j); }
         rc = frameCostMany(jobs);
+        part(0);
         if (rc != X265AMD_OK) return rc;
         jobs.clear();
         for (int b = 1; b < numFrames; b++)
@@ -713,6 +781,7 @@
                 jobs.push_back(j);
             }
         rc = frameCostMany(jobs);
+        part(1);
         if (rc != X265AMD_OK) return rc;
         jobs.clear();
         for (int b = 1; b < numFrames; b++)
@@ -734,6 +803,7 @@
             if (hasL0(frames[numFrames], i) && frames[numFrames]->cost2[i][0] < 0 && frames[numFrames]->specCost2[i][0] < 0)
             { CostJob j; j.fenc = frames[numFrames]; j.ref0 = frames[numFrames - i]; j.d0 = i; j.spec = true; jobs.push_back(j); }
         rc = frameCostMany(jobs);
+        part(2);
         if (rc != X265AMD_OK) return rc;
     }
     const bool isScenecut = p.bHistBasedSceneCut ? histBasedScenecut(frames, 0, 1, origNumFrames) : scenecut(frames, 0, 1, true, origNumFrames, rc);
@@ -817,7 +887,9 @@
         for (int j = 1; j <= numFrames; j++) frames[j]->type = TYPE_P;
         resetStart = bKeyframe ? 1 : 2;
     }
+    part(3);
     if (p.cuTree && (rc = runCuTree(frames, std::min(numFrames, p.keyframeMax), bKeyframe)) != X265AMD_OK) return rc;
+    part(4);
     for (int64_t j = (int64_t)keyintLimit + 1; j <= numFrames; j += p.keyframeMax) { frames[j]->type = TYPE_I; resetStart = std::min(resetStart, (int)j + 1); }
     const int maxp1 = std::min(p.bframes + 1, origNumFrames);
     for (int j = resetStart; j <= numFrames; j++)
@@ -863,6 +935,7 @@
     for (size_t k = 0; k < frames.size(); k++)
     {
         Pic& f = *frames[k];
+        f.needLowres();
         if (f.intraCostHost.empty() || f.qpAqOffset.empty()) return xa_fail(X265AMD_EINVAL, "encoder: cuTree: a picture without block offsets");
         x265amd_cutree_frame& r = recs[k];
         memset(&r, 0, sizeof(r));
@@ -892,6 +965,7 @@
     while ((int)input.size() >= fullQueue && maxGops-- > 0)
     {
         const int maxSearch = std::max(1, std::min(p.lookaheadDepth, 250));
+        for (auto& q : input) { const int rc = lowresFinish(*q); if (rc != X265AMD_OK) return rc; }
         std::vector<Pic*> frames;
         frames.push_back(lastNonB.get());
         for (int j = 0; j < maxSearch && j < (int)input.size(); j++) frames.push_back(input[j].get());
diff --git a/x265-amod_amd/csrc/plane_kernels.hip b/x265-amod_amd/csrc/plane_kernels.hip
--- a/x265-amod_amd/csrc/plane_kernels.hip
+++ b/x265-amod_amd/csrc/plane_kernels.hip
@@ -72,6 +72,17 @@
     for (int x = from + (int)threadIdx.x; x < to; x += blockDim.x) dst[x] = src[min(max(x, 0), width - 1)];
 }
 
+struct InputPic3 { pixel* dst[3]; const unsigned char* src[3]; long dstStride[3], srcStrideBytes[3]; int srcW[3], srcH[3], cols[3], lines[3], marginX[3], marginY[3]; };
+__global__ __launch_bounds__(256) void k_input_picture3(InputPic3 I)
+{
+    const int p = blockIdx.y;
+    if ((int)blockIdx.x >= I.lines[p]) return;
+    const int y = (int)blockIdx.x - I.marginY[p], marginX = I.marginX[p], last = I.srcW[p] - 1, cols = I.cols[p];
+    const pixel* srcRow = (const pixel*)(I.src[p] + (long)min(max(y, 0), I.srcH[p] - 1) * I.srcStrideBytes[p]);
+    pixel* dstRow = I.dst[p] + (long)y * I.dstStride[p] - marginX;
+    for (int i = threadIdx.x; i < cols; i += blockDim.x) dstRow[i] = srcRow[min(max(i - marginX, 0), last)];
+}
+
 __global__ __launch_bounds__(256) void k_weight_plane(const pixel* src, pixel* dst, long stride, int width, int height, int marginX, int marginY,
                                                       int w0, int round, int shift, int offset)
 {
@@ -144,6 +155,34 @@
     return xa_extend_border_band_420(stream, d_y, d_u, d_v, stride, cstride, width, height, marginX, marginY, y_begin, y_end, x_begin, x_end, left, right);
 }
 
+int xa_input_picture_420(void* stream, x265amd_pixel* d_pic, const size_t org[3], size_t pic_elems, intptr_t stride, intptr_t cstride, int width, int height, int marginX, int marginY,
+                         const void* const src[3], const int src_stride_bytes[3], int src_width, int src_height)
+{
+    if (!d_pic || !org || !src || !src_stride_bytes || width <= 0 || height <= 0 || src_width <= 0 || src_height <= 0 || src_width > width || src_height > height ||
+        ((width | height | marginX | marginY | src_width | src_height) & 1) || marginX < 0 || marginY < 0)
+        return xa_fail(X265AMD_EINVAL, "xa_input_picture_420: bad arguments");
+    InputPic3 I;
+    size_t at = 0;
+    for (int p = 0; p < 3; p++)
+    {
+        const int sh = p ? 1 : 0;
+        I.marginX[p] = marginX >> sh; I.marginY[p] = marginY >> sh;
+        I.cols[p] = (width >> sh) + 2 * I.marginX[p]; I.lines[p] = (height >> sh) + 2 * I.marginY[p];
+        I.dstStride[p] = (long)(p ? cstride : stride);
+        I.srcW[p] = src_width >> sh; I.srcH[p] = src_height >> sh;
+        I.src[p] = (const unsigned char*)src[p]; I.srcStrideBytes[p] = src_stride_bytes[p];
+        I.dst[p] = (pixel*)d_pic + org[p];
+        if (!src[p] || src_stride_bytes[p] < (int)(I.srcW[p] * sizeof(pixel)) || I.cols[p] != I.dstStride[p] || org[p] != at + (size_t)I.marginY[p] * I.dstStride[p] + I.marginX[p])
+            return xa_fail(X265AMD_EINVAL, "xa_input_picture_420: the planes do not tile the picture buffer");
+        at += (size_t)I.lines[p] * I.dstStride[p];
+    }
+    if (at != pic_elems) return xa_fail(X265AMD_EINVAL, "xa_input_picture_420: the planes do not tile the picture buffer");
+    hipLaunchKernelGGL(k_input_picture3, dim3(I.lines[0], 3), dim3(256), 0, (hipStream_t)stream, I);
+    hipError_t e = hipGetLastError();
+    if (e != hipSuccess) return xa_fail(X265AMD_EHIP, hipGetErrorString(e));
+    return X265AMD_OK;
+}
+
 extern "C" int x265amd_weight_plane(void* stream, const x265amd_pixel* d_src, x265amd_pixel* d_dst, intptr_t stride, int width, int height,
                                     int marginX, int marginY, int inputWeight, int inputOffset, int log2WeightDenom)
 {
```

After: 104.5. About the same (-0.3%).
